# marekvinkler/NTrace

Measured on AMD Instinct MI355X. Metric: Mrays/sec (primary + 8xAO) on Crytek Sponza, higher is better.
Workload: dtype f32

## Files before the change

### include/ntrace_amd.h

```cpp
#ifndef NTRACE_AMD_H
#define NTRACE_AMD_H

#include <stddef.h>
#include <stdint.h>

#ifdef __cplusplus
extern "C" {
#endif

#define NTR_API __attribute__((visibility("default")))

typedef enum NtrStatus {
    NTR_OK = 0,
    NTR_ERR_INVALID = -1,
    NTR_ERR_NO_DEVICE = -2,
    NTR_ERR_HIP = -3,
    NTR_ERR_LAYOUT = -4,
    NTR_ERR_UNKNOWN_KERNEL = -5,
    NTR_ERR_OVERFLOW = -6,
    NTR_ERR_NOMEM = -7
} NtrStatus;

typedef enum NtrBVHLayout {
    NTR_BVHLayout_AOS_AOS = 0,
// ... 5 lines not shown
    NTR_BVHLayout_CPU,
    NTR_BVHLayout_Max
} NtrBVHLayout;

typedef struct NtrKernelConfig {
    int32_t bvhLayout;
    int32_t blockWidth;
    int32_t blockHeight;
    int32_t usePersistentThreads;
} NtrKernelConfig;

typedef struct NtrRay {
    float ox, oy, oz, tmin;
    float dx, dy, dz, tmax;
} NtrRay;

typedef struct NtrRayResult {
    int32_t id;
    float   t;
    int32_t padA;
    int32_t padB;
} NtrRayResult;


NTR_API const char* ntr_last_error(void);
NTR_API int         ntr_version(void);

NTR_API int ntr_device_count(int* count);
NTR_API int ntr_set_device(int device);
NTR_API int ntr_malloc(void** d_ptr, size_t bytes);
NTR_API int ntr_free(void* d_ptr);
NTR_API int ntr_memcpy_h2d(void* d_dst, const void* h_src, size_t bytes, void* stream);
NTR_API int ntr_memcpy_d2h(void* h_dst, const void* d_src, size_t bytes, void* stream);
NTR_API int ntr_memcpy_d2d(void* d_dst, const void* d_src, size_t bytes, void* stream);
NTR_API int ntr_memset(void* d_dst, int value, size_t bytes, void* stream);
NTR_API int ntr_stream_synchronize(void* stream);


NTR_API int ntr_query_config(const char* kernelName, NtrKernelConfig* config);

NTR_API int ntr_trace_bvh(const char* kernelName, int32_t numRays, int32_t anyHit,
                          const NtrRay* d_rays, NtrRayResult* d_results,
                          const void* d_nodes, int64_t nodesBytes,
                          const void* d_triWoop, int64_t triWoopBytes, const int32_t* d_triIndex,
                          int32_t layout, uint32_t bvhFlags, void* stream, float* seconds);

NTR_API int ntr_trace_status(void* stream, uint32_t* statusBits);

NTR_API int ntr_selftest_gather_rate(int64_t tableBytes, int32_t waves, int32_t lanesPerWave, int32_t steps, void* stream, float* seconds);

NTR_API int ntr_trace_graph_reserve(int32_t launches, int32_t numRays);
NTR_API int ntr_trace_graph_release_all(void);

NTR_API int ntr_stream_release(void* stream);

NTR_API int ntr_selftest_auto_hint_table(int32_t devices, int32_t keysPerDevice, int32_t rounds, int32_t* hintedLastRound);

typedef struct NtrTracePlan {
    int32_t variant;
    int32_t launchVariant;
    int32_t launchBlocks;
    int32_t numBlocks;
    int32_t orderBlocks;
    int32_t chunk, fetchThreshold, leafSwitchBelow, octant, flatFetch, uniformPrologue, splitSlice;
    int32_t numHeads, shardRays, numBlocksIncoherent;
    int32_t numBlocksDivergent;
    int32_t wholeWave;
    int32_t prefetchAfter;
    int32_t unified;
    int32_t minipool;
    int32_t poolKConst;
    int32_t poolKFromDevice;
    int32_t minipoolWide;
    int32_t hintable;
    int32_t useAutoHint;
    int32_t predictable;
    int32_t persistentOrder;
    int32_t probeOnRefresh;
    int32_t coherentRoute;
    int32_t persistentVariant, persistentBlocks, persistentFetchThreshold;
    int32_t perrayBlocks, perrayFetchThreshold;
} NtrTracePlan;
#define NTR_PLAN_FLAG_STATS 1
#define NTR_PLAN_FLAG_CAPTURING 2
#define NTR_PLAN_FLAG_CALLER_HINT 4
NTR_API int ntr_trace_plan(const char* kernelName, int32_t numRays, int32_t anyHit, uint64_t nodesAddr, int64_t nodesBytes,
                           uint64_t triWoopAddr, int64_t triWoopBytes, uint32_t bvhFlags, int32_t numCUs, int32_t flags,
                           NtrTracePlan* plan);
NTR_API int ntr_trace_plan_hint_step(int32_t valid, int32_t predicted, int32_t uses, int32_t out[3]);
NTR_API int ntr_trace_plan_certain(int32_t anyHit, int32_t out[2]);

NTR_API int ntr_tunables_reload(void);

typedef struct NtrSchedHint NtrSchedHint;
NTR_API int ntr_sched_hint_create(NtrSchedHint** out);
NTR_API int ntr_sched_hint_destroy(NtrSchedHint* hint);
NTR_API int ntr_sched_hint_reset(NtrSchedHint* hint);
NTR_API int ntr_trace_bvh_hinted(const char* kernelName, int32_t numRays, int32_t anyHit,
                                 const NtrRay* d_rays, NtrRayResult* d_results,
                                 const void* d_nodes, int64_t nodesBytes,
                                 const void* d_triWoop, int64_t triWoopBytes, const int32_t* d_triIndex,
                                 int32_t layout, uint32_t bvhFlags, void* stream, float* seconds,
                                 NtrSchedHint* hint);

NTR_API int ntr_sched_hint_predict(NtrSchedHint* hint, const uint32_t* d_blockCost, int32_t numBlocks, void* stream);
NTR_API int ntr_bvh_leaf_depths(const void* d_nodes, int64_t nodesBytes, const void* d_triWoop, int64_t triWoopBytes,
                                const int32_t* d_triIndex, int32_t numTris, int32_t* d_depthByTri, int32_t* levels, void* stream);
NTR_API int ntr_secondary_block_costs(const NtrRayResult* d_inResults, int32_t first, int32_t count, int32_t numSamples,
                                      const int32_t* d_depthByTri, int32_t numTris, uint32_t* d_blockCost, void* stream);

NTR_API int ntr_predict_block_costs(int32_t numRays, const NtrRay* d_rays, const void* d_nodes, int64_t nodesBytes,
                                    uint32_t* d_blockCost, void* stream);

NTR_API int ntr_predict_batch_coherence(int32_t numRays, const NtrRay* d_rays, const void* d_nodes, int64_t nodesBytes,
                                        uint32_t* d_out, void* stream);

NTR_API int ntr_predict_dispatch_order(int32_t numRays, const NtrRay* d_rays, const void* d_nodes, int64_t nodesBytes,
                                       uint32_t* d_order, uint32_t* d_word, void* stream);

typedef struct {
    int32_t numBlocks;
    int32_t device;
    int32_t uses;
    int32_t valid;
    int32_t predicted;
} NtrSchedHintState;
NTR_API int ntr_sched_hint_inspect(const NtrSchedHint* hint, NtrSchedHintState* state, uint32_t* h_order, uint32_t* h_cost, void* stream);

typedef struct NtrTraceStats {
    int64_t numRays;
    int64_t numInnerVisits;
    int64_t numTriTests;
    int64_t numLeafVisits;
    int64_t numHits;
} NtrTraceStats;

NTR_API int ntr_trace_bvh_stats(const char* kernelName, int32_t numRays, int32_t anyHit,
                                const NtrRay* d_rays, NtrRayResult* d_results,
                                const void* d_nodes, int64_t nodesBytes,
                                const void* d_triWoop, int64_t triWoopBytes, const int32_t* d_triIndex,
                                int32_t layout, uint32_t bvhFlags, void* stream, NtrTraceStats* stats);

#define NTR_BVH_FINITE 1u
#define NTR_BVH_FASTDIV 2u
#define NTR_BVH_NOTINY 4u
#define NTR_BVH_ORDERED 8u
#define NTR_BVH_WIDE_LEAVES 16u
#define NTR_BATCH_DIVERGENT 0x10000u
NTR_API int ntr_bvh_validate(const void* d_nodes, int64_t nodesBytes, uint32_t* flags, void* stream);

NTR_API int ntr_selftest_division(const float* d_x, int32_t nx, const float* d_d, int32_t nd,
                                  uint32_t* mismatches, void* stream);
NTR_API int ntr_selftest_division_hard(int32_t xExp, int32_t dExp, uint64_t* pairs, uint64_t* mismatches, void* stream);


NTR_API int ntr_pixel_table(int32_t w, int32_t h, int32_t* d_indexToPixel, int32_t* d_pixelToIndex, void* stream);

NTR_API int ntr_raygen_primary(NtrRay* d_rays, int32_t* d_idToSlot, int32_t* d_slotToID,
                               const int32_t* d_indexToPixel, const float origin[3],
                               const float nscreenToWorld[16], int32_t w, int32_t h, float maxDist,
                               uint32_t kernelSeed, void* stream);

NTR_API int ntr_raygen_ao(NtrRay* d_outRays, int32_t* d_outIDToSlot, int32_t* d_outSlotToID,
                          const NtrRay* d_inRays, const NtrRayResult* d_inResults,
                          const float* d_triNormals, int32_t firstInputSlot, int32_t numInputRays,
                          int32_t numSamples, float maxDist, uint32_t kernelSeed, void* stream);

NTR_API int ntr_raygen_ao_normals(NtrRay* d_outRays, int32_t* d_outIDToSlot, int32_t* d_outSlotToID, const NtrRay* d_inRays,
                                  const NtrRayResult* d_inResults, const float* d_rayNormals ,
                                  int32_t firstInputSlot, int32_t numInputRays, int32_t numSamples, float maxDist,
                                  uint32_t kernelSeed, void* stream);

NTR_API int ntr_raygen_shadow(NtrRay* d_outRays, int32_t* d_outIDToSlot, int32_t* d_outSlotToID, const NtrRay* d_inRays,
                              const NtrRayResult* d_inResults, int32_t firstInputSlot, int32_t numInputRays, int32_t numSamples,
                              const float lightPos[3], float lightRadius, uint32_t kernelSeed, void* stream);

NTR_API int ntr_count_hits(const NtrRayResult* d_results, int32_t numRays, int32_t* count, void* stream);


typedef struct NtrLbvhResult {
    int32_t numNodes, numLeaves, numLevels, pad;
    int64_t nodesBytes, triWoopBytes, triIndexBytes;
    float   seconds;
    float   mortonMs, sortMs, woopMs, emitMs, refitMs;
} NtrLbvhResult;

NTR_API int ntr_lbvh_capacity(int32_t numTris, int64_t* nodesBytes, int64_t* triWoopBytes, int64_t* triIndexBytes);

NTR_API int ntr_lbvh_build(int32_t numTris, const int32_t* d_triVtxIndex, int32_t numVerts, const float* d_vtxPos,
                           const float sceneMin[3], const float sceneMax[3], int32_t leafSize, float epsilon,
                           void* d_nodes, int64_t nodesCapacity, void* d_triWoop, int64_t triWoopCapacity,
                           int32_t* d_triIndex, int64_t triIndexCapacity, NtrLbvhResult* result, void* stream);

typedef struct NtrHlbvhResult {
    NtrLbvhResult lbvh;
    int32_t numClusters, topNodes, topLevels, pad;
    float   clusterMs, topMs, bottomMs, pad2;
} NtrHlbvhResult;

NTR_API int ntr_hlbvh_build(int32_t numTris, const int32_t* d_triVtxIndex, int32_t numVerts, const float* d_vtxPos,
                            const float sceneMin[3], const float sceneMax[3], int32_t leafSize, float epsilon, int32_t hlbvhBits,
                            void* d_nodes, int64_t nodesCapacity, void* d_triWoop, int64_t triWoopCapacity,
                            int32_t* d_triIndex, int64_t triIndexCapacity, NtrHlbvhResult* result, void* stream);

NTR_API int ntr_lbvh_release_workspace(void);

typedef struct NtrPersistentBvhParams {
    int32_t triLimit, triMaxLimit, maxDepth, pad;
    float   ci, ct, epsilon, pad2;
} NtrPersistentBvhParams;
typedef struct NtrPersistentBvhResult {
    int32_t numNodes, numLeaves, numLevels, maxDepth;
    int32_t medianFallbacks, costLeaves, depthLeaves, pad;
    int64_t nodesBytes, triWoopBytes, triIndexBytes;
    float   seconds;
    float   prepMs, levelsMs, emitMs;
} NtrPersistentBvhResult;
NTR_API int ntr_persistent_bvh_params_default(NtrPersistentBvhParams* params);
NTR_API int ntr_persistent_bvh_build(int32_t numTris, const int32_t* d_triVtxIndex, int32_t numVerts, const float* d_vtxPos,
                                     const float sceneMin[3], const float sceneMax[3], const NtrPersistentBvhParams* params,
                                     void* d_nodes, int64_t nodesCapacity, void* d_triWoop, int64_t triWoopCapacity,
                                     int32_t* d_triIndex, int64_t triIndexCapacity, NtrPersistentBvhResult* result, void* stream);
NTR_API int ntr_persistent_bvh_scratch_bytes(int64_t* bytes);

typedef struct NtrSahDeviceResult {
    int32_t numNodes, numLeaves, numLevels, maxDepth;
    int32_t numDropped, pad[3];
    int64_t nodesBytes, triWoopBytes, triIndexBytes;
    float   seconds;
    float   prepMs, sortMs, levelsMs, emitMs;
} NtrSahDeviceResult;
NTR_API int ntr_sah_device_build(int32_t numTris, const int32_t* d_triVtxIndex, int32_t numVerts, const float* d_vtxPos,
                                 int32_t minLeafSize, int32_t maxLeafSize, void* d_nodes, int64_t nodesCapacity, void* d_triWoop,
                                 int64_t triWoopCapacity, int32_t* d_triIndex, int64_t triIndexCapacity, NtrSahDeviceResult* result,
                                 void* stream);
NTR_API int ntr_sah_device_scratch_bytes(int64_t* bytes);

#define NTR_PLOC_TAIL 1024
#define NTR_PLOC_TILE 1024
typedef struct NtrPlocResult {
    int32_t numNodes, numLeaves, numRounds, height;
    int32_t tailClusters, pad[3];
    int64_t nodesBytes, triWoopBytes, triIndexBytes;
    float   seconds;
    float   mortonMs, sortMs, roundsMs, tailMs, emitMs;
} NtrPlocResult;
NTR_API int ntr_ploc_build(int32_t numTris, const int32_t* d_triVtxIndex, int32_t numVerts, const float* d_vtxPos,
                           const float sceneMin[3], const float sceneMax[3], int32_t radius, void* d_nodes, int64_t nodesCapacity,
                           void* d_triWoop, int64_t triWoopCapacity, int32_t* d_triIndex, int64_t triIndexCapacity, NtrPlocResult* result,
                           void* stream);
NTR_API int ntr_ploc_scratch_bytes(int64_t* bytes);

typedef struct NtrBlasRange { int64_t nodesOffset, nodesBytes, triWoopOffset, triWoopBytes; } NtrBlasRange;
typedef struct NtrInstance {
    float   objectToWorld[12];
    float   worldToObject[12];
    int32_t blas;
    int32_t reserved[3];
} NtrInstance;
typedef struct NtrTlasResult {
    int32_t rootLink, numNodes, numRounds, height;
    int32_t tailClusters, pad[3];
    int64_t nodesBytes, recordsBytes;
    float   sceneMin[3], sceneMax[3];
    float   seconds;
    float   boxesMs, sortMs, clustersMs, roundsMs, tailMs;
} NtrTlasResult;
NTR_API int ntr_instance_invert(const float objectToWorld[12], float worldToObject[12]);
NTR_API int ntr_tlas_capacity(int32_t numInstances, int64_t* nodesBytes, int64_t* recordsBytes);
NTR_API int ntr_tlas_build(int32_t numInstances, const NtrInstance* d_instances, int32_t numBlas, const NtrBlasRange* blasRanges,
                           const void* d_poolNodes, int64_t poolNodesBytes, int32_t radius, void* d_tlasNodes, int64_t tlasNodesCapacity,
                           void* d_records, int64_t recordsCapacity, NtrTlasResult* result, void* stream);
NTR_API int ntr_tlas_scratch_bytes(int64_t* bytes);
NTR_API int ntr_trace_instanced(int32_t numRays, int32_t anyHit, const NtrRay* d_rays, NtrRayResult* d_results, int32_t* d_instanceIDs,
                                const void* d_tlasNodes, int64_t tlasNodesBytes, int32_t rootLink, const void* d_records,
                                int32_t numInstances, const void* d_poolNodes, int64_t poolNodesBytes, const void* d_poolTriWoop,
                                int64_t poolTriWoopBytes, const int32_t* d_poolTriIndex, float* seconds ,
                                void* stream);

typedef struct NtrInstanceVisibility {
    const uint32_t* d_instanceMasks;
    const uint32_t* d_rayMasks;
    uint32_t rayMask, pad;
} NtrInstanceVisibility;
typedef struct NtrInstancedTraceStats {
    int64_t numRays;
    int64_t numTopInnerVisits;
    int64_t numInstanceEntries;
    int64_t numInstancesMasked;
    int64_t numInnerVisits;
    int64_t numTriTests;
    int64_t numLeafVisits;
    int64_t numHits;
} NtrInstancedTraceStats;
NTR_API int ntr_trace_instanced_masked(int32_t numRays, int32_t anyHit, const NtrRay* d_rays, NtrRayResult* d_results, int32_t* d_instanceIDs,
                                       const void* d_tlasNodes, int64_t tlasNodesBytes, int32_t rootLink, const void* d_records,
                                       int32_t numInstances, const void* d_poolNodes, int64_t poolNodesBytes, const void* d_poolTriWoop,
                                       int64_t poolTriWoopBytes, const int32_t* d_poolTriIndex,
                                       const NtrInstanceVisibility* vis , float* seconds ,
                                       void* stream);
NTR_API int ntr_trace_instanced_stats(int32_t numRays, int32_t anyHit, const NtrRay* d_rays, NtrRayResult* d_results, int32_t* d_instanceIDs,
                                      const void* d_tlasNodes, int64_t tlasNodesBytes, int32_t rootLink, const void* d_records,
                                      int32_t numInstances, const void* d_poolNodes, int64_t poolNodesBytes, const void* d_poolTriWoop,
                                      int64_t poolTriWoopBytes, const int32_t* d_poolTriIndex,
                                      const NtrInstanceVisibility* vis , NtrInstancedTraceStats* stats, void* stream);

// ... 246 lines not shown
```

### ntrace_amd/__init__.py

```python
from ._capi import (BvhView, RAY_DTYPE, RESULT_DTYPE, HostBvh, KernelConfig, NtrError, TraceStats, bvh_validate, lib,
                    lib_path, query_config, sah_build, trace_bvh, trace_bvh_stats, pixel_table,
                    raygen_primary, raygen_ao, raygen_shadow, count_hits, selftest_division, selftest_division_hard, bvh_leaf_depths, secondary_block_costs, lbvh_capacity,
                    lbvh_build, LbvhResult, hlbvh_build, HlbvhResult, reconstruct, ray_morton_sort, camera_decode, camera_reencode,
                    camera_nscreen_to_world, obj_load, SchedHint, trace_status, trace_plan, trace_plan_hint_step, trace_plan_certain, TracePlan, set_tunables, host_bvh_wrap, use_library, trace_graph_reserve, trace_graph_release_all, stream_release, selftest_auto_hint_table, selftest_gather_rate, frame_shard, frame_ao_batches, DistGroup,
                    lbvh_release_workspace, predict_block_costs, predict_batch_coherence, predict_dispatch_order, SchedHintState,
                    HostKdtree, kdtree_build, host_kdtree_wrap, trace_kdtree, KDTREE_SPATIAL_MEDIAN, KDTREE_SAH,
                    DeviceKdtree, KdtreeDeviceParams, kdtree_device_build, kdtree_device_params, KDTREE_DEVICE_DEFAULTS,
                    kdtree_device_scratch_bytes, PersistentBvhParams, PersistentBvhResult, persistent_bvh_params,
                    persistent_bvh_build, persistent_bvh_scratch_bytes, PERSISTENT_BVH_DEFAULTS, SahDeviceResult,
                    sah_device_build, sah_device_scratch_bytes, BvhRefitResult, bvh_refit,
                    bvh_refit_scratch_bytes, BvhOptimizeResult, BvhSahResult, bvh_optimize, bvh_optimize_scratch_bytes, bvh_sah_cost,
                    BvhReorderResult, bvh_reorder, bvh_reorder_scratch_bytes,
                    PlocResult, ploc_build, ploc_scratch_bytes, PLOC_TAIL, PLOC_TILE,
                    PlocBatchMesh, PlocBatchMeshResult, PlocBatchResult, ploc_batch_capacity, ploc_build_batch, ploc_batch_scratch_bytes,
                    RefitBatchEntry, BvhRefitBatchResult, bvh_refit_batch, bvh_refit_batch_scratch_bytes,
                    INSTANCE_DTYPE, BlasRange, BlasPool, TlasResult, instance_invert, make_instances, tlas_capacity, tlas_build,
                    tlas_scratch_bytes, trace_instanced, InstanceVisibility, InstancedTraceStats,
                    trace_instanced_masked, trace_instanced_stats, TlasRefitResult, tlas_refit, tlas_refit_scratch_bytes,
                    BlasTris, BLAS_TRIS_DTYPE, InstancedGeometry, instanced_hit_attributes, raygen_ao_normals,
                    BvhWideResult, bvh_widen_capacity, bvh_widen, bvh_widen_scratch_bytes, trace_wide, trace_wide_stats)

BVHLayout_Compact = 4
BVH_FINITE, BVH_FASTDIV, BVH_NOTINY, BVH_ORDERED, BVH_WIDE_LEAVES = 1, 2, 4, 8, 16
KERNELS = ("fermi_speculative_while_while", "tesla_persistent_while_while",
           "tesla_persistent_speculative_while_while", "kepler_dynamic_fetch")

__all__ = ["BvhView", "RAY_DTYPE", "RESULT_DTYPE", "HostBvh", "KernelConfig", "NtrError", "bvh_validate", "lib",
           "lib_path", "query_config", "sah_build", "trace_bvh", "trace_bvh_stats", "TraceStats", "pixel_table", "raygen_primary", "raygen_ao", "count_hits", "selftest_division", "selftest_division_hard", "bvh_leaf_depths", "secondary_block_costs", "lbvh_capacity", "lbvh_build", "LbvhResult", "hlbvh_build", "HlbvhResult", "reconstruct", "ray_morton_sort", "camera_decode", "camera_reencode", "camera_nscreen_to_world", "obj_load", "SchedHint", "trace_status", "set_tunables", "host_bvh_wrap", "BVHLayout_Compact", "KERNELS",
           "HostKdtree", "kdtree_build", "host_kdtree_wrap", "trace_kdtree", "KDTREE_SPATIAL_MEDIAN", "KDTREE_SAH",
           "DeviceKdtree", "KdtreeDeviceParams", "kdtree_device_build", "kdtree_device_params", "KDTREE_DEVICE_DEFAULTS",
           "kdtree_device_scratch_bytes", "PersistentBvhParams", "PersistentBvhResult", "persistent_bvh_params",
           "persistent_bvh_build", "persistent_bvh_scratch_bytes", "PERSISTENT_BVH_DEFAULTS", "SahDeviceResult",
           "sah_device_build", "sah_device_scratch_bytes", "BvhRefitResult", "bvh_refit",
           "bvh_refit_scratch_bytes", "BvhOptimizeResult", "BvhSahResult", "bvh_optimize", "bvh_optimize_scratch_bytes",
           "bvh_sah_cost", "BvhReorderResult", "bvh_reorder", "bvh_reorder_scratch_bytes",
           "PlocResult", "ploc_build", "ploc_scratch_bytes", "PLOC_TAIL", "PLOC_TILE",
           "PlocBatchMesh", "PlocBatchMeshResult", "PlocBatchResult", "ploc_batch_capacity", "ploc_build_batch", "ploc_batch_scratch_bytes",
           "RefitBatchEntry", "BvhRefitBatchResult", "bvh_refit_batch", "bvh_refit_batch_scratch_bytes",
           "INSTANCE_DTYPE", "BlasRange", "BlasPool", "TlasResult", "instance_invert", "make_instances", "tlas_capacity", "tlas_build",
           "tlas_scratch_bytes", "trace_instanced", "InstanceVisibility", "InstancedTraceStats",
           "trace_instanced_masked", "trace_instanced_stats", "TlasRefitResult", "tlas_refit", "tlas_refit_scratch_bytes",
           "BlasTris", "BLAS_TRIS_DTYPE", "InstancedGeometry", "instanced_hit_attributes", "raygen_ao_normals",
           "BvhWideResult", "bvh_widen_capacity", "bvh_widen", "bvh_widen_scratch_bytes", "trace_wide", "trace_wide_stats"]
```

### ntrace_amd/_capi.py

```python
import ctypes as C
import os

import numpy as np

_HERE = os.path.dirname(os.path.abspath(__file__))

RAY_DTYPE = np.dtype([("ox", "<f4"), ("oy", "<f4"), ("oz", "<f4"), ("tmin", "<f4"),
                      ("dx", "<f4"), ("dy", "<f4"), ("dz", "<f4"), ("tmax", "<f4")])
RESULT_DTYPE = np.dtype([("id", "<i4"), ("t", "<f4"), ("padA", "<i4"), ("padB", "<i4")])


class NtrError(RuntimeError):
    def __init__(self, code, msg):
        super().__init__("ntrace_amd error %d: %s" % (code, msg))
        self.code = code


class SchedHintState(C.Structure):
    _fields_ = [(n, C.c_int32) for n in ("numBlocks", "device", "uses", "valid", "predicted")]


class KernelConfig(C.Structure):
    _fields_ = [("bvhLayout", C.c_int32), ("blockWidth", C.c_int32), ("blockHeight", C.c_int32),
                ("usePersistentThreads", C.c_int32)]
# ... 154 lines not shown
    _fields_ = [("numEntries", C.c_int32), ("lanesPerLeaf", C.c_int32), ("numNodes", C.c_int64), ("numLeaves", C.c_int64),
                ("numRows", C.c_int64), ("firstBadEntry", C.c_int32), ("errBits", C.c_int32), ("seconds", C.c_float), ("pad", C.c_float)]

    def as_dict(self):
        return {k: getattr(self, k) for k, _ in self._fields_ if k != "pad"}


class BlasTris(C.Structure):
    _fields_ = [("firstTri", C.c_int32), ("numTris", C.c_int32)]


BLAS_TRIS_DTYPE = np.dtype([("firstTri", "<i4"), ("numTris", "<i4")])


class InstancedGeometry(C.Structure):
    _fields_ = [("numInstances", C.c_int32), ("numBlas", C.c_int32), ("numTrisTotal", C.c_int32), ("numVerts", C.c_int32),
                ("d_instances", C.c_void_p), ("d_blasTris", C.c_void_p), ("d_triVtxIndex", C.c_void_p), ("d_vtxPos", C.c_void_p)]

    def __init__(self, num_instances=0, num_blas=0, num_tris_total=0, num_verts=0, d_instances=0, d_blas_tris=0, d_tri=0, d_pos=0):
        super().__init__(int(num_instances), int(num_blas), int(num_tris_total), int(num_verts), int(d_instances) or None,
                         int(d_blas_tris) or None, int(d_tri) or None, int(d_pos) or None)


class TlasResult(C.Structure):
    _fields_ = [("rootLink", C.c_int32), ("numNodes", C.c_int32), ("numRounds", C.c_int32), ("height", C.c_int32),
                ("tailClusters", C.c_int32), ("pad", C.c_int32 * 3), ("nodesBytes", C.c_int64), ("recordsBytes", C.c_int64),
                ("sceneMin", C.c_float * 3), ("sceneMax", C.c_float * 3), ("seconds", C.c_float), ("boxesMs", C.c_float),
                ("sortMs", C.c_float), ("clustersMs", C.c_float), ("roundsMs", C.c_float), ("tailMs", C.c_float)]

    def as_dict(self):
        return {k: (list(getattr(self, k)) if k.startswith("scene") else getattr(self, k)) for k, _ in self._fields_ if k != "pad"}


class TlasRefitResult(C.Structure):
    _fields_ = [("numNodes", C.c_int32), ("numLeaves", C.c_int32), ("errBits", C.c_int32), ("pad", C.c_int32),
                ("sceneMin", C.c_float * 3), ("sceneMax", C.c_float * 3), ("seconds", C.c_float), ("pad2", C.c_float)]

    def as_dict(self):
        return {k: (list(getattr(self, k)) if k.startswith("scene") else getattr(self, k)) for k, _ in self._fields_ if not k.startswith("pad")}


class BvhWideResult(C.Structure):
    _fields_ = [("nodesBytes", C.c_int64), ("numNodes", C.c_int32), ("counts", C.c_int32 * 3), ("numLeafLinks", C.c_int32),
                ("height", C.c_int32), ("stackBound", C.c_int32), ("seconds", C.c_float)]

    def as_dict(self):
        return {k: (list(getattr(self, k)) if k == "counts" else getattr(self, k)) for k, _ in self._fields_}


class BvhRefitResult(C.Structure):
    _fields_ = [("numNodes", C.c_int32), ("numLeaves", C.c_int32), ("numRows", C.c_int32), ("pad", C.c_int32), ("seconds", C.c_float)]

    def as_dict(self):
        return {k: getattr(self, k) for k, _ in self._fields_ if k != "pad"}


class BvhOptimizeResult(C.Structure):
    _fields_ = [("passes", C.c_int32), ("numNodes", C.c_int32), ("numLeafLinks", C.c_int32), ("pad", C.c_int32),
                ("formed", C.c_int32 * 8), ("rewritten", C.c_int32 * 8), ("heightBefore", C.c_int32 * 8), ("heightAfter", C.c_int32 * 8),
                ("seconds", C.c_float)]

    def as_dict(self):
        n = self.passes
        return {k: (list(getattr(self, k))[:n] if k in ("formed", "rewritten", "heightBefore", "heightAfter") else getattr(self, k))
                for k, _ in self._fields_ if k != "pad"}


class BvhReorderResult(C.Structure):
    _fields_ = [("nodesBytes", C.c_int64), ("triWoopBytes", C.c_int64), ("triIndexBytes", C.c_int64),
                ("numNodes", C.c_int32), ("numLeaves", C.c_int32), ("numRows", C.c_int32), ("numDroppedSlots", C.c_int32),
                ("seconds", C.c_float)]

    def as_dict(self):
        return {k: getattr(self, k) for k, _ in self._fields_}


class BvhSahResult(C.Structure):
    _fields_ = [("sahCost", C.c_float), ("numNodes", C.c_int32), ("numLeaves", C.c_int32), ("numTris", C.c_int32), ("height", C.c_int32),
                ("seconds", C.c_float)]

    def as_dict(self):
        return {k: getattr(self, k) for k, _ in self._fields_}


class _DeviceKdtreeInfo(C.Structure):
    _fields_ = [("nodes", C.c_void_p), ("nodesBytes", C.c_int64), ("triWoop", C.c_void_p),
                ("triWoopBytes", C.c_int64), ("triIndex", C.c_void_p), ("triIndexBytes", C.c_int64),
                ("sceneMin", C.c_float * 3), ("sceneMax", C.c_float * 3), ("delta", C.c_float),
                ("numInnerNodes", C.c_int32), ("numLeafNodes", C.c_int32), ("numEmptyLeaves", C.c_int32), ("numTriRefs", C.c_int32),
                ("maxDepth", C.c_int32), ("numLevels", C.c_int32), ("percentDuplicates", C.c_float), ("seconds", C.c_float),
                ("prepMs", C.c_float), ("levelsMs", C.c_float), ("emitMs", C.c_float)]


def lib_path():
    return os.environ.get("NTR_LIB_OVERRIDE") or os.path.join(_HERE, "libntrace_amd.so")


_lib = None
_libs = {}

_vp, _i32, _i64, _u32 = C.c_void_p, C.c_int32, C.c_int64, C.c_uint32
SYMBOLS = [
    ("ntr_last_error", C.c_char_p, []),
    ("ntr_version", C.c_int, []),
    ("ntr_device_count", C.c_int, [C.POINTER(C.c_int)]),
    ("ntr_set_device", C.c_int, [C.c_int]),
    ("ntr_malloc", C.c_int, [C.POINTER(_vp), C.c_size_t]),
    ("ntr_free", C.c_int, [_vp]),
    ("ntr_memcpy_h2d", C.c_int, [_vp, _vp, C.c_size_t, _vp]),
    ("ntr_memcpy_d2h", C.c_int, [_vp, _vp, C.c_size_t, _vp]),
    ("ntr_memcpy_d2d", C.c_int, [_vp, _vp, C.c_size_t, _vp]),
    ("ntr_memset", C.c_int, [_vp, C.c_int, C.c_size_t, _vp]),
    ("ntr_stream_synchronize", C.c_int, [_vp]),
    ("ntr_query_config", C.c_int, [C.c_char_p, C.POINTER(KernelConfig)]),
    ("ntr_trace_bvh", C.c_int, [C.c_char_p, _i32, _i32, _vp, _vp, _vp, _i64, _vp, _i64, _vp, _i32, _u32, _vp,
                                C.POINTER(C.c_float)]),
    ("ntr_trace_bvh_hinted", C.c_int, [C.c_char_p, _i32, _i32, _vp, _vp, _vp, _i64, _vp, _i64, _vp, _i32, _u32, _vp,
                                       C.POINTER(C.c_float), _vp]),
    ("ntr_trace_status", C.c_int, [_vp, C.POINTER(_u32)]),
    ("ntr_trace_plan", C.c_int, [C.c_char_p, _i32, _i32, C.c_uint64, _i64, C.c_uint64, _i64, _u32, _i32, _i32, _vp]),
    ("ntr_trace_plan_hint_step", C.c_int, [_i32, _i32, _i32, C.POINTER(_i32 * 3)]),
    ("ntr_trace_plan_certain", C.c_int, [_i32, C.POINTER(_i32 * 2)]),
    ("ntr_selftest_gather_rate", C.c_int, [_i64, _i32, _i32, _i32, _vp, C.POINTER(C.c_float)]),
    ("ntr_frame_shard", C.c_int, [_i32, _i32, _i32, _i32, C.POINTER(_i32), C.POINTER(_i32)]),
    ("ntr_frame_ao_batches", C.c_int, [_i32, _i32, _i32, _i32, C.POINTER(_i32), C.POINTER(_i32), _i32, C.POINTER(_i32)]),
    ("ntr_dist_unique_id", C.c_int, [C.c_char_p]),
    ("ntr_dist_init", C.c_int, [C.c_char_p, _i32, _i32, C.POINTER(_vp)]),
    ("ntr_dist_init_all", C.c_int, [_i32, C.POINTER(_i32), C.POINTER(_vp)]),
    ("ntr_dist_info", C.c_int, [_vp, C.POINTER(_i32), C.POINTER(_i32)]),
    ("ntr_dist_destroy", C.c_int, [_vp]),
    ("ntr_dist_broadcast", C.c_int, [_vp, _vp, _i64, _i32, _vp]),
    ("ntr_dist_broadcast_bvh", C.c_int, [_vp, _vp, _i64, _vp, _i64, _vp, _i64, _i32, _vp]),
    ("ntr_dist_gather_records", C.c_int, [_vp, _vp, _i32, _i32, _vp, _i32, _vp]),
    ("ntr_dist_gather_records_cuts", C.c_int, [_vp, _vp, C.POINTER(_i32), _vp, _i32, _vp]),
    ("ntr_dist_gather_pixels", C.c_int, [_vp, _vp, _vp, _i32, _i32, _vp, _vp, _i32, _vp]),
    ("ntr_tunables_reload", C.c_int, []),
    ("ntr_predict_block_costs", C.c_int, [_i32, _vp, _vp, _i64, _vp, _vp]),
    ("ntr_predict_batch_coherence", C.c_int, [_i32, _vp, _vp, _i64, _vp, _vp]),
    ("ntr_predict_dispatch_order", C.c_int, [_i32, _vp, _vp, _i64, _vp, _vp, _vp]),
    ("ntr_trace_graph_reserve", C.c_int, [_i32, _i32]),
    ("ntr_trace_graph_release_all", C.c_int, []),
    ("ntr_stream_release", C.c_int, [_vp]),
    ("ntr_selftest_auto_hint_table", C.c_int, [_i32, _i32, _i32, C.POINTER(_i32)]),
    ("ntr_lbvh_release_workspace", C.c_int, []),
    ("ntr_sched_hint_create", C.c_int, [C.POINTER(_vp)]),
    ("ntr_sched_hint_destroy", C.c_int, [_vp]),
    ("ntr_sched_hint_reset", C.c_int, [_vp]),
    ("ntr_sched_hint_predict", C.c_int, [_vp, _vp, _i32, _vp]),
    ("ntr_sched_hint_inspect", C.c_int, [_vp, _vp, _vp, _vp, _vp]),
    ("ntr_secondary_block_costs", C.c_int, [_vp, _i32, _i32, _i32, _vp, _i32, _vp, _vp]),
    ("ntr_bvh_leaf_depths", C.c_int, [_vp, _i64, _vp, _i64, _vp, _i32, _vp, C.POINTER(_i32), _vp]),
    ("ntr_selftest_division", C.c_int, [_vp, _i32, _vp, _i32, C.POINTER(_u32), _vp]),
    ("ntr_selftest_division_hard", C.c_int, [_i32, _i32, C.POINTER(C.c_uint64), C.POINTER(C.c_uint64), _vp]),
    ("ntr_trace_bvh_stats", C.c_int, [C.c_char_p, _i32, _i32, _vp, _vp, _vp, _i64, _vp, _i64, _vp, _i32, _u32, _vp,
                                      C.POINTER(TraceStats)]),
    ("ntr_bvh_validate", C.c_int, [_vp, _i64, C.POINTER(_u32), _vp]),
    ("ntr_pixel_table", C.c_int, [_i32, _i32, _vp, _vp, _vp]),
    ("ntr_raygen_primary", C.c_int, [_vp, _vp, _vp, _vp, C.POINTER(C.c_float), C.POINTER(C.c_float), _i32, _i32,
                                     C.c_float, _u32, _vp]),
    ("ntr_raygen_ao", C.c_int, [_vp, _vp, _vp, _vp, _vp, _vp, _i32, _i32, _i32, C.c_float, _u32, _vp]),
    ("ntr_raygen_ao_normals", C.c_int, [_vp, _vp, _vp, _vp, _vp, _vp, _i32, _i32, _i32, C.c_float, _u32, _vp]),
    ("ntr_raygen_shadow", C.c_int, [_vp, _vp, _vp, _vp, _vp, _i32, _i32, _i32, C.POINTER(C.c_float * 3), C.c_float, _u32, _vp]),
    ("ntr_count_hits", C.c_int, [_vp, _i32, C.POINTER(_i32), _vp]),
    ("ntr_lbvh_capacity", C.c_int, [_i32, C.POINTER(_i64), C.POINTER(_i64), C.POINTER(_i64)]),
    ("ntr_lbvh_build", C.c_int, [_i32, _vp, _i32, _vp, C.POINTER(C.c_float), C.POINTER(C.c_float), _i32, C.c_float,
                                 _vp, _i64, _vp, _i64, _vp, _i64, C.POINTER(LbvhResult), _vp]),
    ("ntr_hlbvh_build", C.c_int, [_i32, _vp, _i32, _vp, C.POINTER(C.c_float), C.POINTER(C.c_float), _i32, C.c_float, _i32,
                                  _vp, _i64, _vp, _i64, _vp, _i64, C.POINTER(HlbvhResult), _vp]),
    ("ntr_reconstruct", C.c_int, [_i32, _i32, _i32, _i32, _vp, _vp, _vp, _vp, _vp, _vp, _vp, _vp]),
    ("ntr_ray_morton_sort", C.c_int, [_i32, _vp, _vp, _vp, _vp, _vp, _vp, C.POINTER(C.c_float)]),
    ("ntr_camera_decode", C.c_int, [C.c_char_p, C.POINTER(C.c_float)]),
    ("ntr_camera_reencode", C.c_int, [C.c_char_p, C.c_char_p, _i32]),
    ("ntr_camera_nscreen_to_world", C.c_int, [C.c_char_p, _i32, _i32, C.POINTER(C.c_float), C.POINTER(C.c_float),
                                              C.POINTER(C.c_float)]),
    ("ntr_obj_load", C.c_int, [C.c_char_p, C.POINTER(_vp), C.POINTER(_i32), C.POINTER(_i32), C.POINTER(_i32)]),
    ("ntr_obj_get", C.c_int, [_vp, _vp, _vp]),
    ("ntr_obj_free", None, [_vp]),
    ("ntr_sah_build", C.c_int, [_i32, _vp, _i32, _vp, _i32, _i32, C.POINTER(_vp)]),
    ("ntr_host_bvh_info", C.c_int, [_vp, C.POINTER(_HostBvhInfo)]),
    ("ntr_host_bvh_free", None, [_vp]),
    ("ntr_host_bvh_wrap", C.c_int, [_vp, _i64, _vp, _i64, _vp, _i64, C.POINTER(_vp)]),
    ("ntr_host_bvh_trace", C.c_int, [_vp, _i32, _i32, _vp, _vp, _vp, _i32, C.POINTER(TraceStats)]),
    ("ntr_kdtree_build", C.c_int, [_i32, _i32, _vp, _i32, _vp, _i32, C.POINTER(_vp)]),
    ("ntr_kdtree_device_params_default", C.c_int, [C.POINTER(KdtreeDeviceParams)]),
    ("ntr_kdtree_device_build", C.c_int, [_i32, _vp, _i32, _vp, C.POINTER(KdtreeDeviceParams), C.POINTER(_vp), _vp]),
    ("ntr_device_kdtree_info", C.c_int, [_vp, C.POINTER(_DeviceKdtreeInfo)]),
    ("ntr_device_kdtree_free", None, [_vp]),
    ("ntr_device_kdtree_download", C.c_int, [_vp, _vp, _vp, _vp]),
    ("ntr_kdtree_device_scratch_bytes", C.c_int, [C.POINTER(_i64)]),
    ("ntr_persistent_bvh_params_default", C.c_int, [C.POINTER(PersistentBvhParams)]),
    ("ntr_persistent_bvh_build", C.c_int, [_i32, _vp, _i32, _vp, C.POINTER(C.c_float), C.POINTER(C.c_float), C.POINTER(PersistentBvhParams),
                                           _vp, _i64, _vp, _i64, _vp, _i64, C.POINTER(PersistentBvhResult), _vp]),
    ("ntr_persistent_bvh_scratch_bytes", C.c_int, [C.POINTER(_i64)]),
    ("ntr_sah_device_build", C.c_int, [_i32, _vp, _i32, _vp, _i32, _i32, _vp, _i64, _vp, _i64, _vp, _i64, C.POINTER(SahDeviceResult), _vp]),
    ("ntr_sah_device_scratch_bytes", C.c_int, [C.POINTER(_i64)]),
    ("ntr_ploc_build", C.c_int, [_i32, _vp, _i32, _vp, C.POINTER(C.c_float), C.POINTER(C.c_float), _i32, _vp, _i64, _vp, _i64, _vp, _i64,
                                 C.POINTER(PlocResult), _vp]),
    ("ntr_ploc_scratch_bytes", C.c_int, [C.POINTER(_i64)]),
    ("ntr_instance_invert", C.c_int, [_vp, _vp]),
    ("ntr_ploc_batch_capacity", C.c_int, [_i32, _vp, _vp, C.POINTER(_i64), C.POINTER(_i64), C.POINTER(_i64)]),
    ("ntr_ploc_build_batch", C.c_int, [_i32, _vp, _i32, _vp, _i32, _vp, _i32, _vp, _i64, _vp, _i64, _vp, _i64, _vp, _vp,
                                       C.POINTER(PlocBatchResult), _vp]),
    ("ntr_ploc_batch_scratch_bytes", C.c_int, [C.POINTER(_i64)]),
    ("ntr_tlas_capacity", C.c_int, [_i32, C.POINTER(_i64), C.POINTER(_i64)]),
    ("ntr_tlas_build", C.c_int, [_i32, _vp, _i32, _vp, _vp, _i64, _i32, _vp, _i64, _vp, _i64, C.POINTER(TlasResult), _vp]),
    ("ntr_tlas_scratch_bytes", C.c_int, [C.POINTER(_i64)]),
    ("ntr_tlas_refit", C.c_int, [_i32, _vp, _i32, _vp, _vp, _i64, _vp, _i64, _i32, _vp, _i64, _vp, C.POINTER(TlasRefitResult), _vp]),
    ("ntr_tlas_refit_scratch_bytes", C.c_int, [C.POINTER(_i64)]),
    ("ntr_trace_instanced", C.c_int, [_i32, _i32, _vp, _vp, _vp, _vp, _i64, _i32, _vp, _i32, _vp, _i64, _vp, _i64, _vp, C.POINTER(C.c_float), _vp]),
    ("ntr_trace_instanced_masked", C.c_int, [_i32, _i32, _vp, _vp, _vp, _vp, _i64, _i32, _vp, _i32, _vp, _i64, _vp, _i64, _vp,
                                             C.POINTER(InstanceVisibility), C.POINTER(C.c_float), _vp]),
    ("ntr_trace_instanced_stats", C.c_int, [_i32, _i32, _vp, _vp, _vp, _vp, _i64, _i32, _vp, _i32, _vp, _i64, _vp, _i64, _vp,
                                            C.POINTER(InstanceVisibility), C.POINTER(InstancedTraceStats), _vp]),
    ("ntr_instanced_hit_attributes", C.c_int, [_i32, _vp, _vp, C.POINTER(InstancedGeometry), _vp, _vp, _vp]),
    ("ntr_bvh_widen_capacity", C.c_int, [_i64, C.POINTER(_i64)]),
    ("ntr_bvh_widen", C.c_int, [_vp, _i64, _vp, _i64, C.POINTER(BvhWideResult), _vp]),
    ("ntr_bvh_widen_scratch_bytes", C.c_int, [C.POINTER(_i64)]),
    ("ntr_trace_wide", C.c_int, [_i32, _i32, _vp, _vp, _vp, _i64, _vp, _i64, _vp, _u32, _vp, C.POINTER(C.c_float)]),
    ("ntr_trace_wide_stats", C.c_int, [_i32, _i32, _vp, _vp, _vp, _i64, _vp, _i64, _vp, _u32, _vp, C.POINTER(TraceStats)]),
    ("ntr_bvh_refit", C.c_int, [_vp, _i64, _vp, _i64, _vp, _i64, _i32, _vp, _i32, _vp, C.c_float, _vp, C.POINTER(BvhRefitResult), _vp]),
    ("ntr_bvh_refit_scratch_bytes", C.c_int, [C.POINTER(_i64)]),
    ("ntr_bvh_refit_batch", C.c_int, [_i32, _vp, _vp, _i64, _vp, _i64, _vp, _i32, _vp, _i32, _vp, _vp, C.POINTER(BvhRefitBatchResult), _vp]),
    ("ntr_bvh_refit_batch_scratch_bytes", C.c_int, [C.POINTER(_i64)]),
    ("ntr_bvh_optimize", C.c_int, [_vp, _i64, _i32, C.POINTER(BvhOptimizeResult), _vp]),
    ("ntr_bvh_optimize_scratch_bytes", C.c_int, [C.POINTER(_i64)]),
    ("ntr_bvh_sah_cost", C.c_int, [_vp, _i64, _vp, _i64, C.POINTER(BvhSahResult), _vp]),
    ("ntr_bvh_reorder", C.c_int, [_vp, _i64, _vp, _i64, _vp, _i64, _vp, _i64, _vp, _i64, _vp, _i64, C.POINTER(BvhReorderResult), _vp]),
    ("ntr_bvh_reorder_scratch_bytes", C.c_int, [C.POINTER(_i64)]),
    ("ntr_host_kdtree_info", C.c_int, [_vp, C.POINTER(_HostKdtreeInfo)]),
    ("ntr_host_kdtree_free", None, [_vp]),
    ("ntr_host_kdtree_wrap", C.c_int, [_vp, _i64, _vp, _i64, _vp, _i64, C.POINTER(C.c_float), C.POINTER(C.c_float), C.POINTER(_vp)]),
    ("ntr_trace_kdtree", C.c_int, [_i32, _i32, C.POINTER(C.c_float), C.POINTER(C.c_float), _vp, _vp, _vp, _i64, _vp, _i64, _vp, _i64,
                                   _vp, C.POINTER(C.c_float)]),
]


def _load(path):
    if path not in _libs:
        if not os.path.exists(path):
            raise ImportError("ntrace_amd: %s not found -- run `python -c 'import __graft_entry__ as g; g.build()'` "
                              "(the HIP extension is mandatory; there is no CPU fallback)" % path)
        try:
            import torch
        except ImportError:
            pass
        L = C.CDLL(path)
        for name, res, args in SYMBOLS:
            fn = getattr(L, name)
            fn.restype = res
            fn.argtypes = args
        _libs[path] = L
    return _libs[path]


def lib():
    global _lib
    if _lib is None:
        _lib = _load(lib_path())
    return _lib


def use_library(path=None):
    global _lib
    _lib = _load(path or lib_path())
    return _lib


def _check(rc):
    if rc != 0:
        raise NtrError(rc, (lib().ntr_last_error() or b"").decode("utf-8", "replace"))


def query_config(kernel):
    cfg = KernelConfig()
    _check(lib().ntr_query_config(kernel.encode(), C.byref(cfg)))
    return cfg


class SchedHint:

    def __init__(self):
        self._h = _vp()
        _check(lib().ntr_sched_hint_create(C.byref(self._h)))

    def reset(self):
        _check(lib().ntr_sched_hint_reset(self._h))

    def predict(self, d_block_cost, num_blocks, stream=0):
        _check(lib().ntr_sched_hint_predict(self._h, _vp(d_block_cost), int(num_blocks), _vp(stream)))

    def inspect(self, stream=0):
        st = SchedHintState()
        _check(lib().ntr_sched_hint_inspect(self._h, C.byref(st), None, None, _vp(stream)))
        out = {n: int(getattr(st, n)) for n, _ in st._fields_}
        if st.numBlocks > 0:
            order = np.zeros(st.numBlocks + 3, np.uint32)
            cost = np.zeros(st.numBlocks, np.uint32)
            _check(lib().ntr_sched_hint_inspect(self._h, C.byref(st), order.ctypes.data_as(_vp), cost.ctypes.data_as(_vp), _vp(stream)))
            out.update({n: int(getattr(st, n)) for n, _ in st._fields_})
            out["order"], out["words"], out["cost"] = order[:st.numBlocks], order[st.numBlocks:], cost
        return out

    def close(self):
        if self._h:
            lib().ntr_sched_hint_destroy(self._h)
            self._h = _vp()
# ... 46 lines not shown
    _check(lib().ntr_trace_plan_hint_step(int(bool(valid)), int(bool(predicted)), int(uses), C.byref(out)))
    return dict(zeroK=bool(out[0]), refresh=bool(out[1]), useOrder=bool(out[2]))


def trace_plan_certain(any_hit):
    out = (_i32 * 2)()
    _check(lib().ntr_trace_plan_certain(int(bool(any_hit)), C.byref(out)))
    return dict(certainSteps=bool(out[0]), certainDescent=bool(out[1]))


def trace_status(stream=0):
    bits = _u32(0)
    _check(lib().ntr_trace_status(_vp(stream), C.byref(bits)))
    return int(bits.value)


def selftest_gather_rate(table_bytes, waves, lanes_per_wave=64, steps=256, stream=0):
    sec = C.c_float(0.0)
    _check(lib().ntr_selftest_gather_rate(int(table_bytes), int(waves), int(lanes_per_wave), int(steps), _vp(stream), C.byref(sec)))
    return float(sec.value)


def frame_shard(num_primary, rank, world, align=64):
    lo, hi = _i32(0), _i32(0)
    _check(lib().ntr_frame_shard(int(num_primary), int(rank), int(world), int(align), C.byref(lo), C.byref(hi)))
    return int(lo.value), int(hi.value)


def frame_ao_batches(lo, hi, samples, max_batch_rays):
    n = _i32(0)
    _check(lib().ntr_frame_ao_batches(int(lo), int(hi), int(samples), int(max_batch_rays), None, None, 0, C.byref(n)))
    first, count = (_i32 * max(n.value, 1))(), (_i32 * max(n.value, 1))()
    _check(lib().ntr_frame_ao_batches(int(lo), int(hi), int(samples), int(max_batch_rays), first, count, n.value, C.byref(n)))
    return [(int(first[i]), int(count[i])) for i in range(n.value)]


class DistGroup:

    @staticmethod
    def unique_id():
        buf = C.create_string_buffer(128)
        _check(lib().ntr_dist_unique_id(buf))
        return buf.raw

    def __init__(self, uid, rank, world, _handle=None):
        if _handle is not None:
            self._h, self.rank, self.world = _handle, int(rank), int(world)
            return
        h = _vp()
        _check(lib().ntr_dist_init(C.c_char_p(uid), int(rank), int(world), C.byref(h)))
        self._h, self.rank, self.world = h, int(rank), int(world)

    @staticmethod
    def init_all(devices):
        n = len(devices)
        devs = (_i32 * n)(*[int(x) for x in devices])
        hs = (_vp * n)()
        _check(lib().ntr_dist_init_all(n, devs, hs))
        return [DistGroup(None, i, n, _handle=_vp(hs[i])) for i in range(n)]

    def broadcast(self, d_buf, nbytes, root=0, stream=0):
        _check(lib().ntr_dist_broadcast(self._h, _vp(d_buf), int(nbytes), int(root), _vp(stream)))

    def broadcast_bvh(self, d_nodes, nodes_bytes, d_woop, woop_bytes, d_tri_index, tri_index_bytes, root=0, stream=0):
        _check(lib().ntr_dist_broadcast_bvh(self._h, _vp(d_nodes), int(nodes_bytes), _vp(d_woop), int(woop_bytes), _vp(d_tri_index), int(tri_index_bytes),
                                            int(root), _vp(stream)))

    def gather_records(self, d_own, num_primary, d_full, root=0, stream=0, align=64):
        _check(lib().ntr_dist_gather_records(self._h, _vp(d_own), int(num_primary), int(align), _vp(d_full), int(root), _vp(stream)))

    def gather_records_cuts(self, d_own, cuts, d_full, root=0, stream=0):
        if len(cuts) != self.world + 1:
            raise ValueError("gather_records_cuts: %d cut points for %d ranks" % (len(cuts), self.world))
        c = (_i32 * (self.world + 1))(*[int(x) for x in cuts])
        _check(lib().ntr_dist_gather_records_cuts(self._h, _vp(d_own), c, _vp(d_full), int(root), _vp(stream)))

    def gather_pixels(self, d_own_pixels, d_slot_to_pixel, num_primary, d_full_pixels, d_scratch, root=0, stream=0, align=64):
        _check(lib().ntr_dist_gather_pixels(self._h, _vp(d_own_pixels), _vp(d_slot_to_pixel), int(num_primary), int(align), _vp(d_full_pixels), _vp(d_scratch),
                                            int(root), _vp(stream)))

    def close(self):
        if self._h:
            lib().ntr_dist_destroy(self._h)
            self._h = None


def predict_batch_coherence(num_rays, d_rays, d_nodes, nodes_bytes, d_out, stream=0):
    _check(lib().ntr_predict_batch_coherence(int(num_rays), _vp(d_rays), _vp(d_nodes), int(nodes_bytes), _vp(d_out), _vp(stream)))


def predict_dispatch_order(num_rays, d_rays, d_nodes, nodes_bytes, d_order, d_word, stream=0):
    _check(lib().ntr_predict_dispatch_order(int(num_rays), _vp(d_rays), _vp(d_nodes), int(nodes_bytes), _vp(d_order), _vp(d_word), _vp(stream)))


def predict_block_costs(num_rays, d_rays, d_nodes, nodes_bytes, d_block_cost, stream=0):
    _check(lib().ntr_predict_block_costs(int(num_rays), _vp(d_rays), _vp(d_nodes), int(nodes_bytes), _vp(d_block_cost), _vp(stream)))


def trace_graph_reserve(launches, num_rays):
    _check(lib().ntr_trace_graph_reserve(int(launches), int(num_rays)))


def trace_graph_release_all():
    _check(lib().ntr_trace_graph_release_all())


def stream_release(stream=0):
    _check(lib().ntr_stream_release(_vp(stream)))


def selftest_auto_hint_table(devices, keys_per_device, rounds=3):
    out = (_i32 * devices)()
    _check(lib().ntr_selftest_auto_hint_table(devices, keys_per_device, rounds, out))
    return [int(x) for x in out]


def lbvh_release_workspace():
    _check(lib().ntr_lbvh_release_workspace())


def set_tunables(**kv):
    for k, v in kv.items():
        if v is None:
            os.environ.pop(k, None)
        else:
            os.environ[k] = str(v)
    _check(lib().ntr_tunables_reload())


def bvh_leaf_depths(d_nodes, nodes_bytes, d_woop, woop_bytes, d_tri_index, num_tris, d_depth_by_tri, stream=0):
    m = _i32(0)
    _check(lib().ntr_bvh_leaf_depths(_vp(d_nodes), int(nodes_bytes), _vp(d_woop), int(woop_bytes), _vp(d_tri_index), int(num_tris),
                                     _vp(d_depth_by_tri), C.byref(m), _vp(stream)))
    return int(m.value)


def secondary_block_costs(d_in_results, first, count, num_samples, d_depth_by_tri, num_tris, d_block_cost, stream=0):
    _check(lib().ntr_secondary_block_costs(_vp(d_in_results), int(first), int(count), int(num_samples), _vp(d_depth_by_tri), int(num_tris),
                                           _vp(d_block_cost), _vp(stream)))


def selftest_division(d_x, nx, d_d, nd, stream=0):
    m = _u32(0)
    _check(lib().ntr_selftest_division(_vp(d_x), int(nx), _vp(d_d), int(nd), C.byref(m), _vp(stream)))
    return int(m.value)


def selftest_division_hard(x_exp, d_exp, stream=0):
    n, m = C.c_uint64(0), C.c_uint64(0)
    _check(lib().ntr_selftest_division_hard(int(x_exp), int(d_exp), C.byref(n), C.byref(m), _vp(stream)))
    return int(n.value), int(m.value)


def trace_bvh_stats(kernel, num_rays, any_hit, d_rays, d_results, d_nodes, nodes_bytes, d_woop, woop_bytes,
                    d_tri_index, layout=4, bvh_flags=0, stream=0):
    st = TraceStats()
    _check(lib().ntr_trace_bvh_stats(kernel.encode(), int(num_rays), int(bool(any_hit)), _vp(d_rays), _vp(d_results),
                                     _vp(d_nodes), int(nodes_bytes), _vp(d_woop), int(woop_bytes), _vp(d_tri_index),
                                     int(layout), int(bvh_flags), _vp(stream), C.byref(st)))
    return st


def bvh_validate(d_nodes, nodes_bytes, stream=0):
    flags = _u32(0)
    _check(lib().ntr_bvh_validate(_vp(d_nodes), int(nodes_bytes), C.byref(flags), _vp(stream)))
    return int(flags.value)


def pixel_table(w, h, d_index_to_pixel, d_pixel_to_index=0, stream=0):
    _check(lib().ntr_pixel_table(int(w), int(h), _vp(d_index_to_pixel), _vp(d_pixel_to_index), _vp(stream)))


def raygen_primary(d_rays, d_id_to_slot, d_slot_to_id, d_index_to_pixel, origin, nscreen_to_world, w, h, max_dist,
                   kernel_seed=0, stream=0):
    o = (C.c_float * 3)(*[float(x) for x in origin])
    m = (C.c_float * 16)(*[float(x) for x in np.asarray(nscreen_to_world, dtype=np.float32).reshape(-1)])
    _check(lib().ntr_raygen_primary(_vp(d_rays), _vp(d_id_to_slot), _vp(d_slot_to_id), _vp(d_index_to_pixel), o, m,
                                    int(w), int(h), float(max_dist), int(kernel_seed), _vp(stream)))


def raygen_ao(d_out_rays, d_out_id_to_slot, d_out_slot_to_id, d_in_rays, d_in_results, d_tri_normals, first_input_slot,
              num_input_rays, num_samples, max_dist, kernel_seed=0, stream=0):
    _check(lib().ntr_raygen_ao(_vp(d_out_rays), _vp(d_out_id_to_slot), _vp(d_out_slot_to_id), _vp(d_in_rays),
                               _vp(d_in_results), _vp(d_tri_normals), int(first_input_slot), int(num_input_rays),
                               int(num_samples), float(max_dist), int(kernel_seed), _vp(stream)))


def raygen_ao_normals(d_out_rays, d_out_id_to_slot, d_out_slot_to_id, d_in_rays, d_in_results, d_ray_normals, first_input_slot,
                      num_input_rays, num_samples, max_dist, kernel_seed=0, stream=0):
    _check(lib().ntr_raygen_ao_normals(_vp(d_out_rays), _vp(d_out_id_to_slot), _vp(d_out_slot_to_id), _vp(d_in_rays),
                                       _vp(d_in_results), _vp(d_ray_normals), int(first_input_slot), int(num_input_rays),
                                       int(num_samples), float(max_dist), int(kernel_seed), _vp(stream)))


def raygen_shadow(d_out_rays, d_out_id_to_slot, d_out_slot_to_id, d_in_rays, d_in_results, first_input_slot, num_input_rays, num_samples,
                  light_pos, light_radius, kernel_seed=0, stream=0):
    lp = (C.c_float * 3)(*[float(x) for x in light_pos])
    _check(lib().ntr_raygen_shadow(_vp(d_out_rays), _vp(d_out_id_to_slot), _vp(d_out_slot_to_id), _vp(d_in_rays), _vp(d_in_results),
                                   int(first_input_slot), int(num_input_rays), int(num_samples), C.byref(lp), float(light_radius),
                                   int(kernel_seed), _vp(stream)))


def count_hits(d_results, num_rays, stream=0):
    cnt = _i32(0)
    _check(lib().ntr_count_hits(_vp(d_results), int(num_rays), C.byref(cnt), _vp(stream)))
    return int(cnt.value)


def reconstruct(ray_type, rays_per_primary, first_primary, num_primary, d_primary_slot_to_id, d_primary_results,
                d_batch_id_to_slot, d_batch_results, d_tri_material_color, d_tri_shaded_color, d_pixels, stream=0):
    _check(lib().ntr_reconstruct(int(ray_type), int(rays_per_primary), int(first_primary), int(num_primary),
                                 _vp(d_primary_slot_to_id), _vp(d_primary_results), _vp(d_batch_id_to_slot),
                                 _vp(d_batch_results), _vp(d_tri_material_color), _vp(d_tri_shaded_color), _vp(d_pixels),
                                 _vp(stream)))


def ray_morton_sort(num_rays, d_in_rays, d_in_slot_to_id, d_out_rays, d_out_id_to_slot, d_out_slot_to_id, stream=0):
    sec = C.c_float(0.0)
    _check(lib().ntr_ray_morton_sort(int(num_rays), _vp(d_in_rays), _vp(d_in_slot_to_id), _vp(d_out_rays),
                                     _vp(d_out_id_to_slot), _vp(d_out_slot_to_id), _vp(stream), C.byref(sec)))
    return float(sec.value)


def lbvh_capacity(num_tris):
    a, b, c = _i64(0), _i64(0), _i64(0)
    _check(lib().ntr_lbvh_capacity(int(num_tris), C.byref(a), C.byref(b), C.byref(c)))
    return int(a.value), int(b.value), int(c.value)


def lbvh_build(num_tris, d_tri, num_verts, d_pos, scene_min, scene_max, leaf_size, epsilon, d_nodes, nodes_cap,
               d_woop, woop_cap, d_idx, idx_cap, stream=0):
    res = LbvhResult()
    mn = (C.c_float * 3)(*[float(x) for x in scene_min])
    mx = (C.c_float * 3)(*[float(x) for x in scene_max])
    _check(lib().ntr_lbvh_build(int(num_tris), _vp(d_tri), int(num_verts), _vp(d_pos), mn, mx, int(leaf_size),
                                float(epsilon), _vp(d_nodes), int(nodes_cap), _vp(d_woop), int(woop_cap), _vp(d_idx),
                                int(idx_cap), C.byref(res), _vp(stream)))
    return res


def hlbvh_build(num_tris, d_tri, num_verts, d_pos, scene_min, scene_max, leaf_size, epsilon, hlbvh_bits, d_nodes, nodes_cap,
                d_woop, woop_cap, d_idx, idx_cap, stream=0):
    res = HlbvhResult()
    mn = (C.c_float * 3)(*[float(x) for x in scene_min])
    mx = (C.c_float * 3)(*[float(x) for x in scene_max])
    _check(lib().ntr_hlbvh_build(int(num_tris), _vp(d_tri), int(num_verts), _vp(d_pos), mn, mx, int(leaf_size), float(epsilon),
                                 int(hlbvh_bits), _vp(d_nodes), int(nodes_cap), _vp(d_woop), int(woop_cap), _vp(d_idx), int(idx_cap),
                                 C.byref(res), _vp(stream)))
    return res


PERSISTENT_BVH_DEFAULTS = dict(triLimit=16, triMaxLimit=16, maxDepth=50, ci=1.0, ct=1.0, epsilon=float(np.finfo(np.float32).eps))


def persistent_bvh_params(**kw):
    p = PersistentBvhParams()
    _check(lib().ntr_persistent_bvh_params_default(C.byref(p)))
    for k, v in kw.items():
        if k not in PERSISTENT_BVH_DEFAULTS:
            raise TypeError("unknown persistent BVH parameter %r" % k)
        setattr(p, k, v)
    return p


def persistent_bvh_build(num_tris, d_tri, num_verts, d_pos, scene_min, scene_max, d_nodes, nodes_cap, d_woop, woop_cap, d_idx, idx_cap,
                         params=None, stream=0):
    if isinstance(params, dict):
        params = persistent_bvh_params(**params)
    res = PersistentBvhResult()
    mn = (C.c_float * 3)(*[float(x) for x in scene_min])
    mx = (C.c_float * 3)(*[float(x) for x in scene_max])
    _check(lib().ntr_persistent_bvh_build(int(num_tris), _vp(d_tri), int(num_verts), _vp(d_pos), mn, mx,
                                          C.byref(params) if params is not None else None, _vp(d_nodes), int(nodes_cap), _vp(d_woop),
                                          int(woop_cap), _vp(d_idx), int(idx_cap), C.byref(res), _vp(stream)))
    return res


def persistent_bvh_scratch_bytes():
    v = _i64(0)
    _check(lib().ntr_persistent_bvh_scratch_bytes(C.byref(v)))
    return int(v.value)


def sah_device_build(num_tris, d_tri, num_verts, d_pos, d_nodes, nodes_cap, d_woop, woop_cap, d_idx, idx_cap, min_leaf=1, max_leaf=1,
                     stream=0):
    res = SahDeviceResult()
    _check(lib().ntr_sah_device_build(int(num_tris), _vp(d_tri), int(num_verts), _vp(d_pos), int(min_leaf), int(max_leaf), _vp(d_nodes),
                                      int(nodes_cap), _vp(d_woop), int(woop_cap), _vp(d_idx), int(idx_cap), C.byref(res), _vp(stream)))
    return res


def sah_device_scratch_bytes():
    v = _i64(0)
    _check(lib().ntr_sah_device_scratch_bytes(C.byref(v)))
    return int(v.value)


PLOC_TAIL, PLOC_TILE = 1024, 1024


def ploc_build(num_tris, d_tri, num_verts, d_pos, scene_min, scene_max, d_nodes, nodes_cap, d_woop, woop_cap, d_idx, idx_cap, radius=8,
               stream=0):
    res = PlocResult()
    mn = (C.c_float * 3)(*[float(x) for x in scene_min])
    mx = (C.c_float * 3)(*[float(x) for x in scene_max])
    _check(lib().ntr_ploc_build(int(num_tris), _vp(d_tri), int(num_verts), _vp(d_pos), mn, mx, int(radius), _vp(d_nodes), int(nodes_cap),
# ... 552 lines not shown
```

### ntrace_amd/csrc/ntr_api.cpp

```cpp

#include <hip/hip_runtime.h>

#include <cstdarg>
#include <cstdio>
#include <cstring>
#include <mutex>

#include "ntrace_amd.h"
#include "ntr_internal.h"
#include "compact_bvh.h"
#include "device_scratch.h"
#include "sched_state.h"
#include "trace_kernels.h"
#include "trace_plan.h"

namespace {

thread_local char g_err[512] = "";

}

namespace ntr {

int set_error(int code, const char* fmt, ...)
{
    va_list ap;
    va_start(ap, fmt);
    vsnprintf(g_err, sizeof(g_err), fmt, ap);
    va_end(ap);
    return code;
}

int hip_fail(hipError_t e, const char* what)
{
    int code = (e == hipErrorNoDevice || e == hipErrorInvalidDevice || e == hipErrorInsufficientDriver)
                   ? NTR_ERR_NO_DEVICE : NTR_ERR_HIP;
    return set_error(code, "%s: %s", what, hipGetErrorString(e));
}

bool stream_is_capturing(hipStream_t s)
{
    hipStreamCaptureStatus st = hipStreamCaptureStatusNone;
    if (hipStreamIsCapturing(s, &st) != hipSuccess) { (void)hipGetLastError(); return false; }
    return st != hipStreamCaptureStatusNone;
}

struct KernelInfo {
    const char* name;
    int variant;
    NtrKernelConfig cfg;
};

static const KernelInfo kKernels[] = {
    {"fermi_speculative_while_while", NTR_VARIANT_PERRAY,
     {NTR_BVHLayout_Compact, 64, 1, 0}},
    {"tesla_persistent_while_while", NTR_VARIANT_PERSISTENT,
     {NTR_BVHLayout_Compact, 64, NTR_TRACE_WAVES_PER_BLOCK, 1}},
    {"tesla_persistent_speculative_while_while", NTR_VARIANT_PERSISTENT,
     {NTR_BVHLayout_Compact, 64, NTR_TRACE_WAVES_PER_BLOCK, 1}},
    {"kepler_dynamic_fetch", NTR_VARIANT_PERSISTENT,
     {NTR_BVHLayout_Compact, 64, NTR_TRACE_WAVES_PER_BLOCK, 1}},
};

static const KernelInfo* find_kernel(const char* name)
{
    if (!name) return nullptr;
    for (const KernelInfo& k : kKernels)
        if (strcmp(k.name, name) == 0) return &k;
    return nullptr;
}

static TraceBatchDesc describe_batch(const KernelInfo* k, int32_t numRays, int32_t anyHit, uint64_t nodesAddr, int64_t nodesBytes,
                                     uint64_t woopAddr, int64_t triWoopBytes, uint32_t bvhFlags, bool wantStats, bool capturing,
                                     bool callerHint, int numCUs)
{
    TraceBatchDesc bd;
    bd.variant = k->variant; bd.dynamicFetch = strcmp(k->name, "kepler_dynamic_fetch") == 0;
    bd.numRays = numRays; bd.anyHit = anyHit != 0; bd.bvhFlags = bvhFlags;
    bd.nodesBytes = nodesBytes; bd.triWoopBytes = triWoopBytes;
    bd.nodesAddr = nodesAddr; bd.woopAddr = woopAddr;
    bd.wantStats = wantStats; bd.capturing = capturing; bd.callerHint = callerHint;
    bd.numCUs = numCUs;
    return bd;
}

struct TraceLaunch {
    TraceParams p{};
    TraceParams pp{};
    bool persistentSide = false, perraySide = false;
    NtrSchedHint* hint = nullptr;
    bool refresh = false;
    bool probeCoherence = false;
    TopTable* predTable = nullptr;
    PredictScratch* predScratch = nullptr;
};

static int bind_trace(DeviceState* ds, const Tunables& tun, const TracePlan& pl, bool capturing, int64_t nodesBytes, hipStream_t s,
                      NtrSchedHint* hint, TraceLaunch* L)
{
    TraceParams& p = L->p;
    const int variant = pl.variant, orderBlocks = pl.orderBlocks;
    int rc = NTR_OK;
    if (pl.useAutoHint) {
        rc = auto_hint_get(ds, p.rays, p.nodes, p.numRays, p.anyHit, s, orderBlocks, &hint);
        if (rc != NTR_OK) return rc;
    }
    L->hint = hint;
    if (hint && pl.hintable) {
        if (hint->numBlocks != orderBlocks || hint->device != ds->device) {
            rc = sched_hint_bind(hint, orderBlocks, ds->device, s);
            if (rc != NTR_OK) return rc;
        }
        const HintStep hs = plan_hint_step(tun, hint->valid, hint->predicted, hint->uses);
        if (hs.zeroK) {
            const hipError_t zk = ntr_launch_zero_words(hint->order + orderBlocks, 3, s);
            if (zk != hipSuccess) return hip_fail(zk, "zero_words launch");
        }
        L->refresh = hs.refresh;
        hint->predicted = false;
        hint->uses++;
        if (hs.useOrder) p.order = hint->order;
        if (L->refresh) {
            const hipError_t ze = ntr_launch_zero_words(hint->cost, orderBlocks, s);
            if (ze != hipSuccess) return hip_fail(ze, "zero_words launch");
            p.cost = hint->cost;
        }
    }

    if (pl.predictable && !(hint && hint->valid) && !p.order) {
        rc = top_table_get(ds, p.nodes, nodesBytes, s, false, &L->predTable);
        if (rc != NTR_OK) return rc;
        rc = predict_scratch_get(ds, s, orderBlocks, &L->predScratch);
        if (rc != NTR_OK) return rc;
        if (L->predScratch) p.order = (hint && pl.hintable) ? hint->order : L->predScratch->order;
        else L->predTable = nullptr;
    }

    L->probeCoherence = !L->predScratch && hint && L->refresh && pl.probeOnRefresh;
    if (L->probeCoherence) {
        rc = top_table_get(ds, p.nodes, nodesBytes, s, false, &L->predTable);
        if (rc != NTR_OK) return rc;
    }
    const unsigned int* word = nullptr;
    if (L->predScratch) word = L->predScratch->classCount + NTR_SCHED_PRED_CLASSES + 2;
    else if (hint && pl.hintable && hint->numBlocks == orderBlocks && hint->order) word = hint->order + orderBlocks + 2;
    const bool routed = pl.coherentRoute == 1 && word != nullptr;
    L->persistentSide = variant == NTR_VARIANT_PERSISTENT || routed;
    L->perraySide = variant != NTR_VARIANT_PERSISTENT || routed;
    if ((pl.minipool && pl.poolKFromDevice) || L->persistentSide) p.poolK = word;

    TraceParams& pp = L->pp = p;
    if (L->persistentSide) {
        rc = counter_set_take(ds, capturing, &pp.counter);
        if (rc != NTR_OK) return rc;
        pp.numBlocks = pl.persistentBlocks; pp.numBlocksIncoherent = pl.numBlocksIncoherent; pp.numBlocksDivergent = pl.numBlocksDivergent;
        pp.fetchThreshold = pl.persistentFetchThreshold;
        pp.shardRays = pl.shardRays;
        if (pp.order) {
            pp.orderBlocks = orderBlocks;
            pp.shardRays = ((orderBlocks + pp.numHeads - 1) / pp.numHeads) * 256;
        }
        pp.routeSkip = routed ? NTR_ROUTE_SKIP_COHERENT : 0;
    }
    if (routed) {
        p.routeSkip = NTR_ROUTE_SKIP_INCOHERENT;
        if (variant == NTR_VARIANT_PERSISTENT) { p.fetchThreshold = pl.perrayFetchThreshold; p.poolKConst = 1; }
    }
    return NTR_OK;
}

static int launch_trace(DeviceState* ds, const Tunables& tun, const TracePlan& pl, const TraceLaunch& L, hipStream_t s, float* seconds,
                        NtrTraceStats* stats)
{
    const TraceParams& p = L.p;
    NtrSchedHint* hint = L.hint;
    const int orderBlocks = pl.orderBlocks;
    StreamEvents<2> ev(s);
    if (seconds) {
        NTR_HIP(ev.create());
        NTR_HIP(hipStreamSynchronize(s));
        NTR_HIP(ev.record(0));
    }
    if (L.predScratch) {
        const hipError_t pe = ntr_launch_predict(p.rays, p.numRays, orderBlocks, L.predTable->table, L.predTable->count, L.predScratch->classCount,
                                                 L.predScratch->classList, (hint && pl.hintable) ? hint->order : L.predScratch->order,
                                                 (hint && pl.hintable) ? hint->order + orderBlocks + 2 : nullptr, pl.minipoolWide, s);
        if (pe != hipSuccess) return hip_fail(pe, "predict launch");
    } else if (L.probeCoherence) {
        const hipError_t ce = ntr_launch_coherence(p.rays, p.numRays, orderBlocks, L.predTable->table, L.predTable->count, hint->order + orderBlocks,
                                                  pl.minipoolWide, s);
        if (ce != hipSuccess) return hip_fail(ce, "coherence launch");
    }
    hipError_t le = hipSuccess;
    if (L.persistentSide) {
        le = ntr_launch_zero_words(L.pp.counter, kPoolHeadsMax * 16, s);
        if (le != hipSuccess) return hip_fail(le, "zero_words launch");
        le = ntr_launch_trace(pl.persistentVariant, &L.pp, pl.persistentBlocks, s);
        if (le != hipSuccess) return hip_fail(le, "trace_bvh launch");
    }
    if (L.perraySide) {
        le = pl.variant == NTR_VARIANT_PERSISTENT ? ntr_launch_trace(NTR_VARIANT_PERRAY_UNIFIED_MINI, &p, pl.perrayBlocks, s)
                                                  : ntr_launch_trace(pl.launchVariant, &p, pl.launchBlocks, s);
        if (le != hipSuccess) return hip_fail(le, "trace_bvh launch");
    }
    if (seconds) NTR_HIP(ev.record(1));
    if (L.refresh) {
        le = ntr_launch_sched_order(hint->cost, orderBlocks, tun.schedClasses, hint->order, 1, s);
        if (le != hipSuccess) return hip_fail(le, "sched_order launch");
        hint->valid = true;
    }
    if (seconds) {
        float ms = 0.0f;
        NTR_HIP(ev.elapsed(0, 1, &ms));
        *seconds = ms * 1e-3f;
        unsigned int st = 0;
        const int rc = status_fetch(ds, s, &st);
        if (rc != NTR_OK) return rc;
        if (st & NTR_STATUS_STACK_OVERFLOW) return set_error(NTR_ERR_OVERFLOW, "trace_bvh: traversal stack overflow");
    }
    if (stats) {
        unsigned long long h[4];
        NTR_HIP(hipMemcpyAsync(h, ds->stats, sizeof(h), hipMemcpyDeviceToHost, s));
        NTR_HIP(hipStreamSynchronize(s));
        stats->numRays = p.numRays;
        stats->numInnerVisits = (int64_t)h[0]; stats->numTriTests = (int64_t)h[1]; stats->numLeafVisits = (int64_t)h[2]; stats->numHits = (int64_t)h[3];
    }
    return NTR_OK;
}

static int32_t certain_steps_of(const Tunables& tun, bool anyHit) { return (tun.certainSteps >= 2 || (tun.certainSteps == 1 && anyHit)) ? 1 : 0; }

static int trace_impl(const char* kernelName, int32_t numRays, int32_t anyHit, const NtrRay* d_rays,
                      NtrRayResult* d_results, const void* d_nodes, int64_t nodesBytes, const void* d_triWoop,
                      int64_t triWoopBytes, const int32_t* d_triIndex, int32_t layout, uint32_t bvhFlags,
                      void* stream, float* seconds, NtrTraceStats* stats, NtrSchedHint* hint = nullptr)
{
    if (seconds) *seconds = 0.0f;
    if (stats) memset(stats, 0, sizeof(*stats));
    const KernelInfo* k = find_kernel(kernelName);
    if (!k) return set_error(NTR_ERR_UNKNOWN_KERNEL, "unknown kernel '%s'", kernelName ? kernelName : "(null)");
    if (numRays < 0) return set_error(NTR_ERR_INVALID, "ntr_trace_bvh: numRays < 0");
    if (numRays == 0) return NTR_OK;
    if (!d_nodes || !d_triWoop || !d_triIndex)
        return set_error(NTR_ERR_INVALID, "CudaBVHTracer: No BVH!");
    if (layout != k->cfg.bvhLayout)
        return set_error(NTR_ERR_LAYOUT, "CudaBVHTracer: Incorrect BVH layout!");
    if (!d_rays || !d_results) return set_error(NTR_ERR_INVALID, "ntr_trace_bvh: null ray/result buffer");
    int rc = check_nodes_bytes("ntr_trace_bvh", "node buffer size", nodesBytes);
    if (rc != NTR_OK) return rc;
    if (triWoopBytes < 16 || (triWoopBytes % 16) != 0 || triWoopBytes > 0xFFFFFFFFll)
        return set_error(NTR_ERR_INVALID, "ntr_trace_bvh: triWoop buffer size must be a multiple of 16 in [16, 4 GiB)");

    DeviceState* ds = nullptr;
    rc = current_device_state_ready(&ds);
    if (rc != NTR_OK) return rc;
    hipStream_t s = (hipStream_t)stream;

    const Tunables tun = tunables();
    const TraceBatchDesc bd = describe_batch(k, numRays, anyHit, (uint64_t)d_nodes, nodesBytes, (uint64_t)d_triWoop, triWoopBytes, bvhFlags,
                                             stats != nullptr, stream_is_capturing(s), hint != nullptr, ds->numCUs);
    const TracePlan pl = plan_trace(tun, bd);

    TraceLaunch L;
    TraceParams& p = L.p;
    p.numRays = numRays; p.anyHit = anyHit ? 1 : 0; p.rays = d_rays; p.results = d_results; p.bvhFlags = bvhFlags;
    p.nodes = d_nodes; p.woop = d_triWoop; p.triIndex = d_triIndex; p.nodesBytes = (uint32_t)nodesBytes; p.woopBytes = (uint32_t)triWoopBytes;
    p.status = ds->status; p.stats = ds->stats;
    p.numHeads = pl.numHeads; p.chunk = pl.chunk; p.fetchThreshold = pl.fetchThreshold; p.wholeWave = pl.wholeWave; p.prefetchAfter = pl.prefetchAfter;
    p.flatFetch = pl.flatFetch; p.uniformPrologue = pl.uniformPrologue; p.splitSlice = pl.splitSlice; p.leafSwitchBelow = pl.leafSwitchBelow;
    p.octant = pl.octant; p.poolKConst = pl.poolKConst;
    p.certainSteps = certain_steps_of(tun, anyHit != 0);
    p.certainDescent = tun.certainDescent != 0 ? 1 : 0;
    if (stats) NTR_HIP(hipMemsetAsync(ds->stats, 0, 4 * sizeof(unsigned long long), s));

    rc = bind_trace(ds, tun, pl, bd.capturing, nodesBytes, s, hint, &L);
    if (rc != NTR_OK) return rc;
    return launch_trace(ds, tun, pl, L, s, seconds, stats);
}

}

static int env_int(const char* name, int def)
{
    const char* v = getenv(name);
    return (v && *v) ? atoi(v) : def;
}

namespace ntr {
static Tunables g_tun;
static bool g_tunLoaded = false;
static std::mutex g_tunMu;

static void tunables_load_locked()
{
    Tunables t;
    t.chunk = env_int("NTR_TRACE_CHUNK", 64);
    t.fetchThreshold = env_int("NTR_TRACE_FETCH_THRESHOLD", -1);
    t.leafSwitchBelow = env_int("NTR_TRACE_LEAF_SWITCH", -1);
    t.blocksPerCU = env_int("NTR_TRACE_BLOCKS_PER_CU", 7);
    t.blocksPerCUIncoherent = env_int("NTR_TRACE_BLOCKS_PER_CU_INCOHERENT", 3);
    t.blocksPerCUDivergent = env_int("NTR_TRACE_BLOCKS_PER_CU_DIVERGENT", 4);
    t.octant = env_int("NTR_TRACE_OCTANT", 1);
    t.flatFetch = env_int("NTR_TRACE_FLAT_FETCH", 1);
    t.uniformPrologue = env_int("NTR_TRACE_UNIFORM_PROLOGUE", 1);
    t.certainSteps = env_int("NTR_TRACE_CERTAIN_STEPS", 1);
    t.certainDescent = env_int("NTR_TRACE_CERTAIN_DESCENT", 1);
    t.splitSlice = env_int("NTR_TRACE_SPLIT_SLICE", 8);
    t.wholeWave = env_int("NTR_TRACE_WHOLE_WAVE", 1);
    t.prefetchAfter = env_int("NTR_TRACE_PREFETCH_AFTER", 8);
    t.minipool = env_int("NTR_TRACE_MINIPOOL", -1);
    t.minipoolWide = env_int("NTR_TRACE_MINIPOOL_WIDE", -1);
    t.minipoolThreshold = env_int("NTR_TRACE_MINIPOOL_THRESHOLD", 48);
    t.unified = env_int("NTR_TRACE_UNIFIED", 1);
    t.poolHeads = env_int("NTR_TRACE_POOL_HEADS", 128);
    t.autoHint = env_int("NTR_TRACE_AUTO_HINT", 1);
    t.autoHintMinRays = env_int("NTR_TRACE_AUTO_HINT_MIN_RAYS", 1 << 17);
    t.route = env_int("NTR_TRACE_ROUTE", 1);
    t.persistentHints = env_int("NTR_TRACE_PERSISTENT_HINTS", 1);
    t.predict = env_int("NTR_TRACE_PREDICT", 1);
    t.predictPersistent = env_int("NTR_TRACE_PREDICT_PERSISTENT", 1);
// ... 176 lines not shown

static int query_table(const char* fn, const void* d_nodes, int64_t nodesBytes, hipStream_t s, DeviceState** ds, TopTable** t)
{
    int rc = check_nodes_bytes(fn, "node buffer size", nodesBytes);
    if (rc == NTR_OK) rc = current_device_state(ds, "hipGetDevice(&dev)");
    if (rc == NTR_OK) rc = top_table_get(*ds, d_nodes, nodesBytes, s, false, t);
    return rc;
}

int ntr_predict_block_costs(int32_t numRays, const NtrRay* d_rays, const void* d_nodes, int64_t nodesBytes, uint32_t* d_blockCost, void* stream)
{
    if (numRays < 0) return set_error(NTR_ERR_INVALID, "ntr_predict_block_costs: numRays < 0");
    if (numRays == 0) return NTR_OK;
    if (!d_rays || !d_nodes || !d_blockCost) return set_error(NTR_ERR_INVALID, "ntr_predict_block_costs: null argument");
    DeviceState* ds = nullptr;
    TopTable* t = nullptr;
    const int rc = query_table("ntr_predict_block_costs", d_nodes, nodesBytes, (hipStream_t)stream, &ds, &t);
    if (rc != NTR_OK) return rc;
    const hipError_t e = ntr_launch_predict_costs(d_rays, numRays, (numRays + 255) / 256, t->table, t->count, d_blockCost, (hipStream_t)stream);
    if (e != hipSuccess) return hip_fail(e, "predict_costs launch");
    return NTR_OK;
}

int ntr_predict_batch_coherence(int32_t numRays, const NtrRay* d_rays, const void* d_nodes, int64_t nodesBytes, uint32_t* d_out, void* stream)
{
    if (numRays < 0) return set_error(NTR_ERR_INVALID, "ntr_predict_batch_coherence: numRays < 0");
    if (!d_out) return set_error(NTR_ERR_INVALID, "ntr_predict_batch_coherence: null argument");
    if (numRays > 0 && (!d_rays || !d_nodes)) return set_error(NTR_ERR_INVALID, "ntr_predict_batch_coherence: null argument");
    if (numRays == 0) {
        const unsigned int none[3] = {0u, 0u, 1u};
        NTR_HIP(hipMemcpyAsync(d_out, none, sizeof(none), hipMemcpyHostToDevice, (hipStream_t)stream));
        NTR_HIP(hipStreamSynchronize((hipStream_t)stream));
        return NTR_OK;
    }
    DeviceState* ds = nullptr;
    TopTable* t = nullptr;
    const int rc = query_table("ntr_predict_batch_coherence", d_nodes, nodesBytes, (hipStream_t)stream, &ds, &t);
    if (rc != NTR_OK) return rc;
    const hipError_t e = ntr_launch_coherence(d_rays, numRays, (numRays + 255) / 256, t->table, t->count, d_out, minipool_wide(tunables(), nodesBytes, numRays),
                                              (hipStream_t)stream);
    if (e != hipSuccess) return hip_fail(e, "coherence launch");
    return NTR_OK;
}

int ntr_predict_dispatch_order(int32_t numRays, const NtrRay* d_rays, const void* d_nodes, int64_t nodesBytes, uint32_t* d_order, uint32_t* d_word,
                               void* stream)
{
    if (numRays < 0) return set_error(NTR_ERR_INVALID, "ntr_predict_dispatch_order: numRays < 0");
    if (numRays == 0) return NTR_OK;
    if (!d_rays || !d_nodes || !d_order || !d_word) return set_error(NTR_ERR_INVALID, "ntr_predict_dispatch_order: null argument");
    hipStream_t s = (hipStream_t)stream;
    DeviceState* ds = nullptr;
    TopTable* t = nullptr;
    int rc = query_table("ntr_predict_dispatch_order", d_nodes, nodesBytes, s, &ds, &t);
    if (rc != NTR_OK) return rc;
    std::lock_guard<std::mutex> lk(ds->queryMu);
    const int numBlocks = (numRays + 255) / 256;
    PredictScratch* p = &ds->query;
    if (p->capBlocks < numBlocks && p->classList) NTR_HIP(hipStreamSynchronize(s));
    rc = scratch_alloc(p, numBlocks);
    if (rc != NTR_OK) return rc;
    const hipError_t e = ntr_launch_predict(d_rays, numRays, numBlocks, t->table, t->count, p->classCount, p->classList, d_order, d_word,
                                            minipool_wide(tunables(), nodesBytes, numRays), s);
    if (e != hipSuccess) return hip_fail(e, "predict launch");
    NTR_HIP(hipStreamSynchronize(s));
    return NTR_OK;
}

int ntr_secondary_block_costs(const NtrRayResult* d_inResults, int32_t first, int32_t count, int32_t numSamples, const int32_t* d_depthByTri,
                              int32_t numTris, uint32_t* d_blockCost, void* stream)
{
    if (first < 0 || count < 0 || numSamples < 1 || numTris < 0 || (count > 0 && (!d_inResults || !d_depthByTri || !d_blockCost)))
        return set_error(NTR_ERR_INVALID, "ntr_secondary_block_costs: bad argument");
    if (count == 0) return NTR_OK;
    hipStream_t s = (hipStream_t)stream;
    const int64_t blocks = ((int64_t)count * numSamples + 255) / 256;
    if (blocks > 0x7FFFFFFF) return set_error(NTR_ERR_INVALID, "ntr_secondary_block_costs: batch too large");
    hipError_t e = ntr_launch_zero_words(d_blockCost, (int)blocks, s);
    if (e == hipSuccess) e = ntr_launch_secondary_block_costs(d_inResults, first, count, numSamples, d_depthByTri, numTris, d_blockCost, s);
    if (e != hipSuccess) return hip_fail(e, "secondary_block_costs launch");
    return NTR_OK;
}

int ntr_bvh_leaf_depths(const void* d_nodes, int64_t nodesBytes, const void* d_triWoop, int64_t triWoopBytes, const int32_t* d_triIndex,
                        int32_t numTris, int32_t* d_depthByTri, int32_t* maxDepth, void* stream)
{
    if (maxDepth) *maxDepth = 0;
    if (!d_nodes || nodesBytes < 64 || (nodesBytes % 64) != 0 || nodesBytes > kMaxNodesBytes || !d_triWoop || triWoopBytes < 16 || !d_triIndex ||
        numTris < 1 || !d_depthByTri)
        return set_error(NTR_ERR_INVALID, "ntr_bvh_leaf_depths: bad argument");
    hipStream_t s = (hipStream_t)stream;
    const unsigned int capacity = (unsigned int)(nodesBytes / 64);
    unsigned int* d_q = nullptr;
    NTR_HIP(hipMalloc((void**)&d_q, (2 * (size_t)capacity + 2) * sizeof(unsigned int)));
    unsigned int* q[2] = {d_q, d_q + capacity};
    unsigned int* cnt = d_q + 2 * (size_t)capacity;
    hipError_t e = hipMemsetAsync(d_depthByTri, 0, (size_t)numTris * sizeof(int32_t), s);
    const unsigned int init[3] = {0u, 1u, 0u};
    if (e == hipSuccess) e = hipMemcpyAsync(q[0], &init[0], sizeof(unsigned int), hipMemcpyHostToDevice, s);
    if (e == hipSuccess) e = hipMemcpyAsync(cnt, &init[1], 2 * sizeof(unsigned int), hipMemcpyHostToDevice, s);
    int depth = 0;
    unsigned long long bound = 1;
    unsigned int frontier = 1;
    while (e == hipSuccess && frontier > 0 && depth < 4096) {
        const int in = depth & 1, out = in ^ 1;
        e = ntr_launch_zero_words(cnt + out, 1, s);
        const unsigned int threads = (unsigned int)(bound < capacity ? bound : capacity);
        if (e == hipSuccess)
            e = ntr_launch_leaf_depth_level(d_nodes, (unsigned int)nodesBytes, d_triWoop, (unsigned int)(triWoopBytes / 16), d_triIndex, numTris, q[in], cnt + in,
                                            q[out], cnt + out, capacity, threads, depth, d_depthByTri, s);
        depth++;
        bound = bound < capacity ? bound * 2 : bound;
        if ((depth & 3) == 0 && e == hipSuccess) {
            e = hipMemcpyAsync(&frontier, cnt + (depth & 1), sizeof(frontier), hipMemcpyDeviceToHost, s);
            if (e == hipSuccess) e = hipStreamSynchronize(s);
            if (frontier > capacity) frontier = capacity;
        }
    }
    if (e == hipSuccess) e = hipStreamSynchronize(s);
    (void)hipFree(d_q);
    if (e != hipSuccess) return hip_fail(e, "ntr_bvh_leaf_depths");
    if (depth >= 4096) return set_error(NTR_ERR_INVALID, "ntr_bvh_leaf_depths: the tree is deeper than 4096 levels (a cycle in the child references?)");
    if (maxDepth) *maxDepth = depth;
    return NTR_OK;
}

int ntr_trace_bvh_stats(const char* kernelName, int32_t numRays, int32_t anyHit, const NtrRay* d_rays,
                        NtrRayResult* d_results, const void* d_nodes, int64_t nodesBytes, const void* d_triWoop,
                        int64_t triWoopBytes, const int32_t* d_triIndex, int32_t layout, uint32_t bvhFlags,
                        void* stream, NtrTraceStats* stats)
{
    if (!stats) return set_error(NTR_ERR_INVALID, "ntr_trace_bvh_stats: null stats");
    return trace_impl(kernelName, numRays, anyHit, d_rays, d_results, d_nodes, nodesBytes, d_triWoop, triWoopBytes,
                      d_triIndex, layout, bvhFlags, stream, nullptr, stats);
}

int ntr_selftest_division(const float* d_x, int32_t nx, const float* d_d, int32_t nd, uint32_t* mismatches, void* stream)
{
    if (!mismatches || !d_x || !d_d || nx <= 0 || nd <= 0) return set_error(NTR_ERR_INVALID, "ntr_selftest_division: bad argument");
    hipStream_t s = (hipStream_t)stream;
    unsigned int* d_m = nullptr;
    NTR_HIP(hipMalloc((void**)&d_m, sizeof(unsigned int)));
    NTR_HIP(hipMemsetAsync(d_m, 0, sizeof(unsigned int), s));
    hipError_t le = ntr_launch_selftest_division(d_x, d_d, nx, nd, d_m, s);
    if (le != hipSuccess) return hip_fail(le, "selftest launch");
    unsigned int m = 0;
    NTR_HIP(hipMemcpyAsync(&m, d_m, sizeof(m), hipMemcpyDeviceToHost, s));
    NTR_HIP(hipStreamSynchronize(s));
    NTR_HIP(hipFree(d_m));
    *mismatches = m;
    return NTR_OK;
}

int ntr_selftest_division_hard(int32_t xExp, int32_t dExp, uint64_t* pairs, uint64_t* mismatches, void* stream)
{
    if (!pairs || !mismatches || xExp < -84 || xExp > 51 || dExp < -40 || dExp > 16)
        return set_error(NTR_ERR_INVALID, "ntr_selftest_division_hard: bad argument (x exponents in [-84, 51], d exponents in [-40, 16])");
    hipStream_t s = (hipStream_t)stream;
    unsigned long long* d_c = nullptr;
    NTR_HIP(hipMalloc((void**)&d_c, 2 * sizeof(unsigned long long)));
    hipError_t e = hipMemsetAsync(d_c, 0, 2 * sizeof(unsigned long long), s);
    if (e == hipSuccess) e = ntr_launch_selftest_division_hard(xExp, dExp, d_c, s);
    unsigned long long h[2] = {0, 0};
    if (e == hipSuccess) e = hipMemcpyAsync(h, d_c, sizeof(h), hipMemcpyDeviceToHost, s);
    if (e == hipSuccess) e = hipStreamSynchronize(s);
    (void)hipFree(d_c);
    if (e != hipSuccess) return hip_fail(e, "ntr_selftest_division_hard");
    *pairs = h[0];
    *mismatches = h[1];
    return NTR_OK;
}

}
```

### ntrace_amd/csrc/selftest_kernels.hip

```cpp
#include <hip/hip_runtime.h>
#include <stdint.h>

#include "trace_kernels.h"
#include "trace_arith.h"

namespace ntr {

__global__ __launch_bounds__(256) void selftest_division_kernel(const float* __restrict__ x, const float* __restrict__ d,
                                                                int nx, int nd, unsigned int* __restrict__ mismatches)
{
    const int i = blockIdx.x * blockDim.x + threadIdx.x;
    if (i >= nx) return;
    const float xv = x[i];
    unsigned int bad = 0;
    for (int j = 0; j < nd; j++) {
        const float dv = d[j];
        const float q0 = xv / dv;
        const float q1 = fast_div(xv, dv, exact_rcp(dv));
        bad += (__float_as_uint(q0) != __float_as_uint(q1)) && !(q0 == 0.0f && q1 == 0.0f);
    }
    if (bad) atomicAdd(mismatches, bad);
}

__global__ __launch_bounds__(256) void selftest_division_hard_kernel(int xe0, int de0, unsigned long long* __restrict__ counts)
{
    const unsigned int D = (1u << 23) + blockIdx.x * 256u + threadIdx.x;
    const int k = __builtin_ctz(D);
    unsigned long long tested = 0, bad = 0;
    if (k <= 3) {
        const unsigned int Dp = D >> k;
        unsigned int inv = Dp;
        for (int it = 0; it < 5; it++) inv *= 2u - Dp * inv;
        for (int b = 24; b <= 25; b++) {
            const unsigned long long mod = 1ull << (b - k);
            for (int Np = -8; Np <= 8; Np++) {
                const long long N = (long long)Np * (1ll << k);
                if (Np == 0 || N > 8 || N < -8) continue;
                const unsigned long long base = ((unsigned long long)(unsigned int)(-Np) * inv) & (mod - 1ull);
                for (unsigned int j = 0; j < (1u << k); j++) {
                    unsigned long long Mo = base + j * mod;
                    while (Mo < (1ull << 24)) Mo += 1ull << b;
                    if (Mo >= (1ull << 25) || !(Mo & 1ull)) continue;
                    const long long num = (long long)((unsigned long long)D * Mo) + N;
                    if (num & ((1ll << b) - 1ll)) continue;
                    const long long X = num >> b;
                    if (b == 24 ? (X < (long long)D || X >= (1ll << 24)) : (X < (1ll << 23) || X >= (long long)D)) continue;
                    for (int e = 0; e < 16; e++) {
                        const float xv = ldexpf((float)X, xe0 + (e & 3) - 23), dv = ldexpf((float)D, de0 + (e >> 2) - 23);
                        for (int sgn = 0; sgn < 2; sgn++) {
                            const float dd = sgn ? -dv : dv;
                            const float q0 = xv / dd;
                            const float q1 = fast_div(xv, dd, exact_rcp(dd));
                            tested++;
                            bad += __float_as_uint(q0) != __float_as_uint(q1);
                        }
                    }
                }
            }
        }
    }
    if (tested) atomicAdd(&counts[0], tested);
    if (bad) atomicAdd(&counts[1], bad);
}

}

extern "C" hipError_t ntr_launch_selftest_division(const float* d_x, const float* d_d, int nx, int nd,
                                                   unsigned int* d_mismatches, hipStream_t stream)
{
    hipLaunchKernelGGL(ntr::selftest_division_kernel, dim3((nx + 255) / 256), dim3(256), 0, stream, d_x, d_d, nx, nd, d_mismatches);
    return hipGetLastError();
}

extern "C" hipError_t ntr_launch_selftest_division_hard(int xe0, int de0, unsigned long long* d_counts, hipStream_t stream)
{
    hipLaunchKernelGGL(ntr::selftest_division_hard_kernel, dim3((1u << 23) / 256u), dim3(256), 0, stream, xe0, de0, d_counts);
    return hipGetLastError();
}
```

### ntrace_amd/csrc/trace_fetch.h

```cpp
#pragma once
#include <hip/hip_runtime.h>
#include <stdint.h>

#include "trace_kernels.h"
#include "compact_bvh.h"

namespace ntr {

typedef __amdgpu_buffer_rsrc_t Rsrc;
typedef unsigned int u32x4 __attribute__((ext_vector_type(4)));
constexpr unsigned int kFetchBytes = kNodeBytes;

__device__ __forceinline__ Rsrc make_rsrc(const void* p, unsigned int bytes)
{
    return __builtin_amdgcn_make_buffer_rsrc(const_cast<void*>(p), 0, (int)bytes, 0x00020000);
}
__device__ __forceinline__ float4 as_f4(u32x4 v) { return make_float4(__uint_as_float(v.x), __uint_as_float(v.y), __uint_as_float(v.z), __uint_as_float(v.w)); }
__device__ __forceinline__ u32x4 as_u4(const float4& f) { return u32x4{__float_as_uint(f.x), __float_as_uint(f.y), __float_as_uint(f.z), __float_as_uint(f.w)}; }
__device__ __forceinline__ float4 ld4(Rsrc r, int byteOfs) { return as_f4(__builtin_amdgcn_raw_buffer_load_b128(r, byteOfs, 0, 0)); }
__device__ __forceinline__ unsigned int ld1(Rsrc r, int byteOfs)
{
    return __builtin_amdgcn_raw_buffer_load_b32(r, byteOfs, 0, 0);
}

__device__ __forceinline__ u32x4 rsrc_words(const void* p, unsigned int bytes)
{
    const unsigned long long a = (unsigned long long)p;
    u32x4 w;
    w.x = __builtin_amdgcn_readfirstlane((unsigned int)a);
    w.y = __builtin_amdgcn_readfirstlane((unsigned int)(a >> 32) & 0xFFFFu);
    w.z = __builtin_amdgcn_readfirstlane(bytes);
    w.w = 0x00020000u;
    return w;
}

#define NTR_FETCH64_TWO_BUFFERS_TEXT                                        \
    "s_mov_b64 %[sav], exec\n\t"                                            \
    "s_and_b64 exec, %[sav], %[ma]\n\t"                                     \
    "buffer_load_dwordx4 %[a], %[ofs], %[ra], 0 offen\n\t"                  \
    "buffer_load_dwordx4 %[b], %[ofs], %[ra], 0 offen offset:16\n\t"        \
    "buffer_load_dwordx4 %[c], %[ofs], %[ra], 0 offen offset:32\n\t"        \
    "buffer_load_dwordx4 %[d], %[ofs], %[ra], 0 offen offset:48\n\t"        \
    "s_and_b64 exec, %[sav], %[mb]\n\t"                                     \
    "buffer_load_dwordx4 %[a], %[ofs], %[rb], 0 offen\n\t"                  \
    "buffer_load_dwordx4 %[b], %[ofs], %[rb], 0 offen offset:16\n\t"        \
    "buffer_load_dwordx4 %[c], %[ofs], %[rb], 0 offen offset:32\n\t"        \
    "buffer_load_dwordx4 %[d], %[ofs], %[rb], 0 offen offset:48\n\t"        \
    "s_mov_b64 exec, %[sav]\n\t"                                            \
    "s_waitcnt vmcnt(0)"
#define NTR_FETCH64_TWO_BUFFERS_INPUTS [ofs] "v"(ofs), [ra] "s"(rsrcA), [rb] "s"(rsrcB), [ma] "s"(maskA), [mb] "s"(maskB)

__device__ __forceinline__ void fetch64_two_buffers(u32x4 rsrcA, u32x4 rsrcB, int ofs, unsigned long long maskA,
                                                    unsigned long long maskB, float4& a, float4& b, float4& c, float4& d)
{
    u32x4 va, vb, vc, vd;
    unsigned long long sav;
    asm volatile(NTR_FETCH64_TWO_BUFFERS_TEXT
                 : [a] "=&v"(va), [b] "=&v"(vb), [c] "=&v"(vc), [d] "=&v"(vd), [sav] "=&s"(sav)
                 : NTR_FETCH64_TWO_BUFFERS_INPUTS
                 : "memory", "scc");
    a = as_f4(va); b = as_f4(vb); c = as_f4(vc); d = as_f4(vd);
}

__device__ __forceinline__ void fetch64_two_buffers_into(u32x4 rsrcA, u32x4 rsrcB, int ofs, unsigned long long maskA,
                                                         unsigned long long maskB, float4& a, float4& b, float4& c, float4& d)
{
    u32x4 va = as_u4(a), vb = as_u4(b), vc = as_u4(c), vd = as_u4(d);
    unsigned long long sav;
    asm volatile(NTR_FETCH64_TWO_BUFFERS_TEXT
                 : [a] "+v"(va), [b] "+v"(vb), [c] "+v"(vc), [d] "+v"(vd), [sav] "=&s"(sav)
                 : NTR_FETCH64_TWO_BUFFERS_INPUTS
                 : "memory", "scc");
    a = as_f4(va); b = as_f4(vb); c = as_f4(vc); d = as_f4(vd);
}
#undef NTR_FETCH64_TWO_BUFFERS_TEXT
#undef NTR_FETCH64_TWO_BUFFERS_INPUTS

struct UnifiedBufs {
    const char* nodes; const char* woop;
    unsigned int nodesBytes, woopBytes;
    u32x4 rNodes, rWoop;
    bool uniformPrologue;
    bool certainSteps;
    bool certainDescent;
    const char* base;
    unsigned int dN, dW;
    unsigned int limNode;
    int limTri;
    unsigned int oddBase, oddSpan;
};
template <bool TRIM = false>
__device__ __forceinline__ UnifiedBufs unified_bufs(const TraceParams& p)
{
    UnifiedBufs u;
    u.nodes = (const char*)p.nodes; u.woop = (const char*)p.woop;
    u.nodesBytes = p.nodesBytes; u.woopBytes = p.woopBytes;
    u.rNodes = rsrc_words(p.nodes, p.nodesBytes); u.rWoop = rsrc_words(p.woop, p.woopBytes);
    u.uniformPrologue = p.uniformPrologue != 0;
    u.certainSteps = p.certainSteps != 0 && (p.bvhFlags & NTR_BVH_ORDERED) != 0;
    u.certainDescent = p.certainDescent != 0;
    const unsigned long long an = (unsigned long long)p.nodes, aw = (unsigned long long)p.woop;
    const unsigned long long lo = an < aw ? an : aw;
    u.base = (const char*)lo;
    u.dN = (unsigned int)(an - lo); u.dW = (unsigned int)(aw - lo);
    u.limNode = p.nodesBytes - kFetchBytes;
    u.limTri = leaf_link((int)((p.woopBytes - kFetchBytes) >> kRowShift));
    u.oddBase = u.limNode + 1u; u.oddSpan = (unsigned)u.limTri - u.oddBase;
    if (TRIM) asm volatile("" : "+s"(u.oddBase), "+s"(u.oddSpan));
    return u;
}

template <bool FLAT, bool TRIM = false>
__device__ __forceinline__ void unified_fetch(const UnifiedBufs& ub, int node, unsigned long long live, float4& a, float4& b, float4& c, float4& d)
{
    const bool inner = (unsigned)node < (unsigned)kSentinel;
    const bool atTri = node < 0;
    if (FLAT) {
        asm volatile("" : "=v"(a.x), "=v"(a.y), "=v"(a.z), "=v"(a.w), "=v"(b.x), "=v"(b.y), "=v"(b.z), "=v"(b.w));
        asm volatile("" : "=v"(c.x), "=v"(c.y), "=v"(c.z), "=v"(c.w), "=v"(d.x), "=v"(d.y), "=v"(d.z), "=v"(d.w));
        const bool okNode = (unsigned)node <= ub.limNode, okTri = TRIM ? (unsigned)node >= (unsigned)ub.limTri : atTri && node >= ub.limTri;
        const bool flatOk = okNode || okTri;
        const unsigned int cofs = okNode ? ub.dN + (unsigned)node : ub.dW + ((unsigned)leaf_row(node) << kRowShift);
        if (flatOk) {
            typedef const __attribute__((address_space(1))) u32x4* global_u4_ptr;
            const global_u4_ptr q = (global_u4_ptr)((const __attribute__((address_space(1))) char*)ub.base + cofs);
            const u32x4 qa = q[0], qb = q[1], qc = q[2], qd = q[3];
            a = as_f4(qa); b = as_f4(qb); c = as_f4(qc); d = as_f4(qd);
        }
        if (TRIM) {
            const unsigned long long odd = live & __builtin_amdgcn_ballot_w64((unsigned)node - ub.oddBase < ub.oddSpan);
            if (__builtin_expect(odd != 0ull, 0))
                fetch64_two_buffers_into(ub.rNodes, ub.rWoop, inner ? node : leaf_row(node) * kRowBytes, odd & __builtin_amdgcn_ballot_w64(inner),
                                         odd & __builtin_amdgcn_ballot_w64(atTri), a, b, c, d);
        } else {
            const unsigned long long odd = __ballot((inner || atTri) && !flatOk);
            if (odd != 0ull)
                fetch64_two_buffers_into(ub.rNodes, ub.rWoop, inner ? node : leaf_row(node) * kRowBytes, __ballot(inner && !flatOk), __ballot(atTri && !flatOk), a, b, c, d);
        }
    } else {
        const int ofs = inner ? node : leaf_row(node) * kRowBytes;
        fetch64_two_buffers(ub.rNodes, ub.rWoop, ofs, __ballot(inner), __ballot(atTri), a, b, c, d);
    }
}

}
```

### ntrace_amd/csrc/trace_kernels.h

```cpp
#pragma once
#include <hip/hip_runtime.h>
#include <stdint.h>

#include "ntrace_amd.h"

#ifndef NTR_TRACE_WAVES_PER_BLOCK
#define NTR_TRACE_WAVES_PER_BLOCK 4
#endif
#ifndef NTR_TRACE_MIN_WAVES_PER_SIMD
#define NTR_TRACE_MIN_WAVES_PER_SIMD 1
#endif
#ifndef NTR_TRACE_PERSISTENT_MIN_WAVES_PER_SIMD
#define NTR_TRACE_PERSISTENT_MIN_WAVES_PER_SIMD 1
#endif

#define NTR_VARIANT_PERRAY 0
#define NTR_VARIANT_PERSISTENT 1
#define NTR_VARIANT_PERRAY_STATS 2
#define NTR_VARIANT_PERSISTENT_UNIFIED 5
#define NTR_VARIANT_PERRAY_UNIFIED_W1 6
#define NTR_MINIPOOL_MAX_K 16
#define NTR_VARIANT_PERRAY_UNIFIED_MINI 7

#define NTR_ROUTE_SKIP_COHERENT 1
#define NTR_ROUTE_SKIP_INCOHERENT 2
#define NTR_BATCH_WORD_K(w) ((w) & 0xFFFFu)
#define NTR_BATCH_WORD_INCOHERENT(w) (NTR_BATCH_WORD_K(w) > 1u || ((w) & NTR_BATCH_DIVERGENT) != 0u)

#define NTR_STATUS_STACK_OVERFLOW 1u


namespace ntr {

struct TraceParams {
    int32_t numRays;
    int32_t anyHit;
    const NtrRay* rays;
    NtrRayResult* results;
    const void* nodes;
    const void* woop;
    uint32_t nodesBytes;
    uint32_t woopBytes;
    const int32_t* triIndex;
    int32_t* counter;
    unsigned int* status;
    int32_t chunk;
    int32_t shardRays;
    int32_t numHeads;
    int32_t numBlocks;
    int32_t numBlocksIncoherent;
    int32_t numBlocksDivergent;
    int32_t orderBlocks;
    int32_t fetchThreshold;
    int32_t wholeWave;
    int32_t prefetchAfter;
    uint32_t bvhFlags;
    int32_t leafSwitchBelow;
    int32_t octant;
    int32_t flatFetch;
    int32_t uniformPrologue;
    int32_t certainSteps;
    int32_t certainDescent;
    int32_t splitSlice;
    const unsigned int* order;
    unsigned int* cost;
    unsigned long long* stats;
    const unsigned int* poolK;
    int32_t poolKConst;
    int32_t routeSkip;
};

}

extern "C" hipError_t ntr_launch_trace(int variant, const ntr::TraceParams* p, int numBlocks, hipStream_t stream);
#define NTR_TOP_DEPTH_MAX 10
#define NTR_SCHED_PRED_CLASSES 64
#define NTR_SCHED_PRED_WORDS (NTR_SCHED_PRED_CLASSES + 3)
extern "C" hipError_t ntr_launch_top_table(const void* d_nodes, unsigned int nodesBytes, int depth, void* d_table,
                                           unsigned int* d_tableCount, hipStream_t stream);
extern "C" hipError_t ntr_launch_predict(const void* d_rays, int numRays, int numBlocks, const void* d_table,
                                         const unsigned int* d_tableCount, unsigned int* d_classCount, unsigned int* d_classList,
                                         unsigned int* d_order, unsigned int* d_poolKCopy, int poolKWide, hipStream_t stream);
extern "C" hipError_t ntr_launch_predict_costs(const void* d_rays, int numRays, int numBlocks, const void* d_table,
                                               const unsigned int* d_tableCount, unsigned int* d_blockCost, hipStream_t stream);
extern "C" hipError_t ntr_launch_coherence(const void* d_rays, int numRays, int numBlocks, const void* d_table, const unsigned int* d_tableCount,
                                           unsigned int* d_out, int poolKWide, hipStream_t stream);
extern "C" hipError_t ntr_launch_leaf_depth_level(const void* d_nodes, unsigned int nodesBytes, const void* d_woop, unsigned int woopVec4, const int* d_triIndex,
                                                  int numTris, const unsigned int* d_qin, const unsigned int* d_nIn, unsigned int* d_qout, unsigned int* d_nOut,
                                                  unsigned int capacity, unsigned int gridThreads, int depth, int* d_depthByTri, hipStream_t stream);
extern "C" hipError_t ntr_launch_secondary_block_costs(const void* d_inResults, int first, int count, int numSamples, const int* d_depthByTri, int numTris,
                                                       unsigned int* d_blockCost, hipStream_t stream);
extern "C" hipError_t ntr_launch_zero_words(void* d_ptr, int words, hipStream_t stream);
extern "C" hipError_t ntr_launch_status_exchange(unsigned int* d_status, unsigned int* d_out, hipStream_t stream);
extern "C" hipError_t ntr_launch_sched_order(const unsigned int* d_cost, int numBlocks, int classes, unsigned int* d_order,
                                             int keepIfAllZero, hipStream_t stream);
extern "C" hipError_t ntr_launch_identity_order(unsigned int* d_order, int numBlocks, hipStream_t stream);
extern "C" hipError_t ntr_launch_selftest_division(const float* d_x, const float* d_d, int nx, int nd,
                                                   unsigned int* d_mismatches, hipStream_t stream);
extern "C" hipError_t ntr_launch_selftest_division_hard(int xe0, int de0, unsigned long long* d_counts, hipStream_t stream);
```

### ntrace_amd/csrc/trace_kernels.hip

```cpp

#include <hip/hip_runtime.h>
#include <stdint.h>

#include "trace_kernels.h"
#include "trace_lane.h"
#include "trace_fetch.h"
#include "trace_prologue.h"
#include "trace_split.h"

namespace ntr {

template <bool FAST, bool STATS, bool DYNAMIC_FETCH, bool SLICED = false>
__device__ __forceinline__ void traverse(Rsrc nodes, Rsrc woop, RayRegs& r, int& node,
                                         LaneStack& st, int (&spill)[SPILL_DEPTH], bool anyHit,
                                         int& hitAddr, float& hitU, float& hitV, LaneStats& ls, unsigned int* status,
                                         bool poolEmpty, int fetchThreshold, int leafSwitchBelow, int* slice = nullptr)
{
    unsigned long long live = __ballot(node != kSentinel);
    while (live != 0ull) {
        if (SLICED && --*slice < 0) break;
        for (;;) {
            const bool inner = (unsigned)node < (unsigned)kSentinel;
            const unsigned long long innerMask = __ballot(inner);
            if (innerMask == 0ull) break;
            if (__popcll(innerMask) < leafSwitchBelow && __ballot(node < 0) != 0ull) break;
            inner_step<FAST>(nodes, inner, r, node, st, spill, status);
            if (STATS && inner) ls.inner++;
        }
        if (node < 0) {
            if (leaf_step<STATS>(woop, r, node, anyHit, hitAddr, hitU, hitV, ls)) node = kSentinel;
            else node = stack_pop(st, spill);
        }
        live = __ballot(node != kSentinel);
        if (DYNAMIC_FETCH && !poolEmpty && __popcll(live) < fetchThreshold) break;
    }
}

template <bool FAST, bool FLAT, int OCT = 8, bool PROLOGUE = false, bool SLICED = false, bool TRIM = false>
__device__ __forceinline__ void traverse_unified(const UnifiedBufs& ub, RayRegs& r, int& node, LaneStack& st,
                                                 int (&spill)[SPILL_DEPTH], bool anyHit, int& hitAddr, float& hitU, float& hitV,
                                                 unsigned int* status, bool poolEmpty, int fetchThreshold, int* slice = nullptr)
{
    if (PROLOGUE && ub.uniformPrologue) uniform_prologue<FAST, OCT, true>(ub, r, node, st, spill, status);
    for (;;) {
        const unsigned long long live = __ballot(node != kSentinel);
        if (live == 0ull) break;
        if (!poolEmpty && __popcll(live) < fetchThreshold) break;
        if (SLICED && --*slice < 0) break;
        float4 a, b, c, d;
        unified_fetch<FLAT, TRIM>(ub, node, live, a, b, c, d);
        if (FLAT && TRIM) { keep_row(a); keep_row(b); keep_row(c); keep_row(d); }
        else if (FLAT) { keep(a); keep(b); keep(c); keep(d); }
        unified_advance<FAST, OCT, LDS_DEPTH, TRIM>(a, b, c, d, r, node, st, spill, anyHit, hitAddr, hitU, hitV, status);
    }
}
__device__ __forceinline__ bool start_ray(const TraceParams& p, int rayIdx, RayRegs& r, int& node, LaneStack& st,
                                          int& hitAddr, float& hitU, float& hitV)
{
    load_ray(p.rays, rayIdx, r);
    hitAddr = -1;
    hitU = hitV = 0.0f;
    stack_reset(st);
    node = (r.tmin < r.tmax) ? 0 : kSentinel;
    return ray_is_nice(r, p.bvhFlags);
}

__device__ __forceinline__ void fresh_prologue(bool fastWave, const UnifiedBufs& ub, const RayRegs& r, int& node, LaneStack& st,
                                               int (&spill)[SPILL_DEPTH], unsigned int* status)
{
    if (fastWave) uniform_prologue<true, 8>(ub, r, node, st, spill, status);
    else uniform_prologue<false, 8>(ub, r, node, st, spill, status);
}

template <bool FLATF>
__device__ __forceinline__ void minipool_body(const TraceParams& p, unsigned int K, lds_int* stackBase);

#define NTR_PERRAY_BOUNDS(W) __launch_bounds__((W) * 64, NTR_TRACE_MIN_WAVES_PER_SIMD)
template <int WAVES, bool STATS, bool UNIFIED = false, bool FLATF = true, bool MINI = false>
__device__ __forceinline__ void perray_body(const TraceParams& p)
{
    __shared__ int s_stack[WAVES][LDS_DEPTH][64];
    if constexpr (MINI) {
        static_assert(WAVES == 1 && UNIFIED && !STATS, "the mini-pool shares the one-wave unified-step launch");
        unsigned int K = (unsigned int)p.poolKConst;
        if (p.poolK) {
            const unsigned int word = *p.poolK;
            if (p.routeSkip == NTR_ROUTE_SKIP_INCOHERENT && NTR_BATCH_WORD_INCOHERENT(word)) return;
            K = NTR_BATCH_WORD_K(word);
        }
        bool pooled = K >= 2u && K <= (unsigned int)NTR_MINIPOOL_MAX_K;
        if (pooled) {
            minipool_body<FLATF>(p, K, (lds_int*)&s_stack[0][0][threadIdx.x]);
            return;
        }
    }
    const int lane = threadIdx.x & 63, wave = threadIdx.x >> 6;
    constexpr int PARTS = 4 / WAVES;
    const unsigned int g = blockIdx.x / PARTS, part = blockIdx.x % PARTS;
    const unsigned int block = p.order ? p.order[g] : g;
    const int rayIdx = block * 256 + part * (WAVES * 64) + threadIdx.x;
    const bool valid = rayIdx < p.numRays;
    const Rsrc nodes = make_rsrc(p.nodes, p.nodesBytes), woop = make_rsrc(p.woop, p.woopBytes);

    unsigned long long tl0 = 0;
    if (p.cost) tl0 = __builtin_amdgcn_s_memrealtime();

    RayRegs r;
    load_ray(p.rays, valid ? rayIdx : 0, r);
    LaneStack st;
    int spill[SPILL_DEPTH];
    st.lds = (lds_int*)&s_stack[wave][0][lane];
    stack_reset(st);

    int hitAddr = -1;
    float hitU = 0.0f, hitV = 0.0f;
    int node = (valid && r.tmin < r.tmax) ? 0 : kSentinel;
    LaneStats ls = {0u, 0u, 0u};

    const bool fastWave = (p.bvhFlags & NTR_BVH_FASTDIV) && __ballot(node != kSentinel && !ray_is_nice(r, p.bvhFlags)) == 0ull;
    int oct = 8;
    if (UNIFIED && fastWave && p.octant && (p.bvhFlags & NTR_BVH_ORDERED)) {
        const unsigned long long liveMask = __ballot(node != kSentinel);
        const unsigned long long sx = __ballot(node != kSentinel && r.dx < 0.0f), sy = __ballot(node != kSentinel && r.dy < 0.0f),
                                 sz = __ballot(node != kSentinel && r.dz < 0.0f);
        if ((sx == 0ull || sx == liveMask) && (sy == 0ull || sy == liveMask) && (sz == 0ull || sz == liveMask))
            oct = (sx ? 1 : 0) | (sy ? 2 : 0) | (sz ? 4 : 0);
    }
    if (UNIFIED) {
        const UnifiedBufs ub = unified_bufs<true>(p);
#define NTR_UNIFIED_OCT(O) traverse_unified<true, FLATF, O, true, false, true>(ub, r, node, st, spill, p.anyHit != 0, hitAddr, hitU, hitV, p.status, true, 0)
        if (oct < 8) {
            switch (oct) {
                case 0: NTR_UNIFIED_OCT(0); break;
                case 1: NTR_UNIFIED_OCT(1); break;
                case 2: NTR_UNIFIED_OCT(2); break;
                case 3: NTR_UNIFIED_OCT(3); break;
                case 4: NTR_UNIFIED_OCT(4); break;
                case 5: NTR_UNIFIED_OCT(5); break;
                case 6: NTR_UNIFIED_OCT(6); break;
                default: NTR_UNIFIED_OCT(7); break;
            }
        }
#undef NTR_UNIFIED_OCT
        else if (fastWave) traverse_unified<true, FLATF, 8, true, false, true>(ub, r, node, st, spill, p.anyHit != 0, hitAddr, hitU, hitV, p.status, true, 0);
        else traverse_unified<false, FLATF, 8, true, false, true>(ub, r, node, st, spill, p.anyHit != 0, hitAddr, hitU, hitV, p.status, true, 0);
    } else if (fastWave) traverse<true, STATS, false>(nodes, woop, r, node, st, spill, p.anyHit != 0, hitAddr, hitU, hitV, ls, p.status, true, 0, p.leafSwitchBelow);
    else traverse<false, STATS, false>(nodes, woop, r, node, st, spill, p.anyHit != 0, hitAddr, hitU, hitV, ls, p.status, true, 0, p.leafSwitchBelow);

    if (p.cost && lane == 0)
        atomicMax(&p.cost[block], (unsigned int)(__builtin_amdgcn_s_memrealtime() - tl0));
    if (!valid) return;
    store_result(p.results, p.triIndex, rayIdx, hitAddr, r.tmax, hitU, hitV);
    if (STATS) {
        atomicAdd(&p.stats[0], (unsigned long long)ls.inner);
        atomicAdd(&p.stats[1], (unsigned long long)ls.tris);
        atomicAdd(&p.stats[2], (unsigned long long)ls.leaves);
        atomicAdd(&p.stats[3], (unsigned long long)(hitAddr >= 0));
    }
}

template <int WAVES, bool STATS, bool UNIFIED = false, bool FLATF = true>
__global__ NTR_PERRAY_BOUNDS(WAVES) void trace_bvh_perray(TraceParams p)
{
    perray_body<WAVES, STATS, UNIFIED, FLATF, false>(p);
}
#define NTR_MINI_BOUNDS __launch_bounds__(64)
__global__ NTR_MINI_BOUNDS void trace_bvh_perray_mini(TraceParams p)
{
    perray_body<1, false, true, true, true>(p);
}
__global__ NTR_MINI_BOUNDS void trace_bvh_perray_mini_desc(TraceParams p)
{
    perray_body<1, false, true, false, true>(p);
}

template <int WAVES, bool UNIFIED = false, bool FLATF = true>
__global__ __launch_bounds__(WAVES * 64, NTR_TRACE_PERSISTENT_MIN_WAVES_PER_SIMD) void trace_bvh_persistent(TraceParams p)
{
    __shared__ int s_stack[WAVES][LDS_DEPTH][64];
    const int lane = threadIdx.x & 63, wave = threadIdx.x >> 6;
    const Rsrc nodes = make_rsrc(p.nodes, p.nodesBytes), woop = make_rsrc(p.woop, p.woopBytes);
    const bool anyHit = p.anyHit != 0;
    const bool bvhFast = (p.bvhFlags & NTR_BVH_FASTDIV) != 0;
    int numBlocksEff = p.numBlocks;
    const unsigned int batchWord = p.poolK ? *p.poolK : 1u;
    const bool incoherentBatch = NTR_BATCH_WORD_INCOHERENT(batchWord);
    if (p.routeSkip == NTR_ROUTE_SKIP_COHERENT && !incoherentBatch) return;
    const int gridIncoherent = NTR_BATCH_WORD_K(batchWord) > 1u ? p.numBlocksIncoherent : p.numBlocksDivergent;
    if (incoherentBatch && gridIncoherent > 0 && gridIncoherent < numBlocksEff) numBlocksEff = gridIncoherent;
    if ((int)blockIdx.x >= numBlocksEff) return;

    LaneStack st;
    int spill[SPILL_DEPTH];
    st.lds = (lds_int*)&s_stack[wave][0][lane];
    stack_reset(st);

    RayRegs r = {0, 0, 0, 0, 0, 0, 0, 0, 0, 0, 0};
    int node = kSentinel, rayIdx = -1, hitAddr = -1;
    float hitU = 0.0f, hitV = 0.0f;
    bool nice = true;
    int chunkNext = 0, chunkEnd = 0;
    bool poolEmpty = false;
    const int numHeads = p.numHeads;
    int shard = (int)(blockIdx.x % (unsigned)numHeads);
    bool firstChunk = true;
    const unsigned int* const order = p.order;
    const int poolEnd = numHeads * p.shardRays;
    auto range_beg = [&](int h) { return h * p.shardRays; };
    int chunkDelta = 0;
    auto chunk_delta = [&](int base, int h) {
        const int off = base - h * p.shardRays;
        if (!order) return ((off / p.chunk) * numHeads + h) * p.chunk - base;
        const int q = (off >> 8) * numHeads + h;
        if (q >= p.orderBlocks) return 0x3FFFFFFF - base;
        return (int)order[q] * 256 + (off & 255) - base;
    };
    auto static_rays = [&](int h) { return ((numBlocksEff - h + numHeads - 1) / numHeads) * WAVES * p.chunk; };
    LaneStats ls = {0u, 0u, 0u};
    SplitState split;
    split_reset(split);
    bool splitOn = false;
    const int splitSlice = UNIFIED ? p.splitSlice : 0;

    const bool dynamicFetch = p.fetchThreshold > 0 && (!UNIFIED || p.wholeWave == 0 || incoherentBatch);
    int prefetched = 0;
    bool havePrefetch = false;
    int prefetchHead = 0;
    int prefetchIn = -1;
    int costBlock = -1;
    unsigned long long costT0 = 0;

    auto grab = [&]() -> bool {
        bool got = false;
        auto take = [&](int base, int h) {
            const int rangeBeg = range_beg(h);
            const int rangeEnd = min(rangeBeg + p.shardRays, poolEnd);
            if (base >= rangeEnd) return false;
            chunkNext = base;
            chunkEnd = min(base + p.chunk, rangeEnd);
            chunkDelta = chunk_delta(base, h);
            return true;
        };
        if (firstChunk) {
            firstChunk = false;
            got = take(range_beg(shard) + ((int)(blockIdx.x / (unsigned)numHeads) * WAVES + __builtin_amdgcn_readfirstlane(wave)) * p.chunk, shard);
        } else if (havePrefetch) {
            havePrefetch = false;
            got = take(__builtin_amdgcn_readfirstlane(prefetched) + static_rays(prefetchHead) + range_beg(prefetchHead), prefetchHead);
        }
        while (!got) {
            int base = 0;
            if (lane == 0) base = atomicAdd(p.counter + shard * 16, p.chunk);
            if (take(__builtin_amdgcn_readfirstlane(base) + static_rays(shard) + range_beg(shard), shard)) { got = true; break; }
            unsigned long long live = 0ull;
            int ofs = 1;
            for (; ofs < numHeads && live == 0ull; ofs += 64) {
                bool has = false;
                if (ofs + lane < numHeads) {
                    const int h = (shard + ofs + lane) % numHeads;
                    const int hb = range_beg(h);
                    const int he = min(hb + p.shardRays, poolEnd);
                    const int taken = __hip_atomic_load(p.counter + h * 16, __ATOMIC_RELAXED, __HIP_MEMORY_SCOPE_AGENT);
                    has = hb + static_rays(h) + taken < he;
                }
                live = __ballot(has);
            }
            if (live == 0ull) break;
            shard = (shard + ofs - 64 + (int)__builtin_ctzll(live)) % numHeads;
        }
        if (got) prefetchIn = p.prefetchAfter;
        return got;
    };
    auto cost_open = [&]() {
        costBlock = (chunkEnd - p.chunk + chunkDelta) >> 8;
        if ((unsigned)costBlock >= (unsigned)((p.numRays + 255) >> 8)) costBlock = -1;
        costT0 = __builtin_amdgcn_s_memrealtime();
    };

    for (;;) {
        unsigned long long empty = __ballot(rayIdx < 0);
        const bool wholeWave = empty == ~0ull;
        const bool refill = !poolEmpty && (wholeWave || (dynamicFetch && 64 - __popcll(empty) < p.fetchThreshold));
        while (refill && empty != 0ull && !poolEmpty) {
            if (chunkNext >= chunkEnd && !grab()) { poolEmpty = true; break; }
            const int prefix = lane_rank(empty);
            const int avail = chunkEnd - chunkNext;
            const int pos = chunkNext + prefix + chunkDelta;
            if (rayIdx < 0 && prefix < avail && pos < p.numRays) {
                rayIdx = pos;
                nice = start_ray(p, rayIdx, r, node, st, hitAddr, hitU, hitV);
            }
            chunkNext += min(__popcll(empty), avail);
            empty = __ballot(rayIdx < 0);
            if (wholeWave && !dynamicFetch) break;
        }
        const bool fresh = refill && wholeWave;
        if (p.cost && refill && wholeWave && !dynamicFetch && !poolEmpty) cost_open();

        if (UNIFIED && poolEmpty && splitSlice > 0) {
            if (!splitOn) { splitOn = true; split_reset(split); }
            split_donate(split, r, node, st, rayIdx, hitAddr, hitU, hitV, nice);
        }
        const bool fastWave = bvhFast && __ballot(node != kSentinel && !nice) == 0ull;
        int slice = 0x7FFFFFFF;
        if (splitOn) slice = splitSlice;
        else if (prefetchIn >= 0 && !poolEmpty) slice = prefetchIn;
        const int fetchBelow = dynamicFetch ? p.fetchThreshold : 0;
        if (UNIFIED) {
            const UnifiedBufs ub = unified_bufs(p);
            if (fresh && p.uniformPrologue) fresh_prologue(fastWave, ub, r, node, st, spill, p.status);
            if (fastWave) traverse_unified<true, FLATF, 8, false, true>(ub, r, node, st, spill, anyHit, hitAddr, hitU, hitV, p.status, poolEmpty, fetchBelow, &slice);
            else traverse_unified<false, FLATF, 8, false, true>(ub, r, node, st, spill, anyHit, hitAddr, hitU, hitV, p.status, poolEmpty, fetchBelow, &slice);
            if (splitOn) split_settle(split, r, node, st, hitAddr, hitU, hitV, anyHit);
        } else {
            if (fresh && p.uniformPrologue) fresh_prologue(fastWave, unified_bufs(p), r, node, st, spill, p.status);
            if (fastWave) traverse<true, false, true, true>(nodes, woop, r, node, st, spill, anyHit, hitAddr, hitU, hitV, ls, p.status, poolEmpty, fetchBelow, p.leafSwitchBelow, &slice);
            else traverse<false, false, true, true>(nodes, woop, r, node, st, spill, anyHit, hitAddr, hitU, hitV, ls, p.status, poolEmpty, fetchBelow, p.leafSwitchBelow, &slice);
        }
        if (!splitOn && prefetchIn >= 0 && !poolEmpty) {
            prefetchIn = -1;
            if (!havePrefetch && __ballot(node != kSentinel) != 0ull) {
                if (lane == 0) prefetched = atomicAdd(p.counter + shard * 16, p.chunk);
                havePrefetch = true;
                prefetchHead = shard;
            }
        }

        if (rayIdx >= 0 && node == kSentinel && (!splitOn || split.base == 0)) {
            store_result(p.results, p.triIndex, rayIdx, hitAddr, r.tmax, hitU, hitV);
            rayIdx = -1;
        }
        if (costBlock >= 0 && __ballot(rayIdx >= 0) == 0ull) {
            if (lane == 0) atomicMax(&p.cost[costBlock], (unsigned int)(__builtin_amdgcn_s_memrealtime() - costT0));
            costBlock = -1;
        }
        if (poolEmpty && __ballot(rayIdx >= 0) == 0ull) break;
    }
}

template <bool FLATF>
__device__ __forceinline__ void minipool_body(const TraceParams& p, unsigned int K, lds_int* stackBase)
{
    const int lane = threadIdx.x;
    const unsigned int numChunks = gridDim.x;
    const unsigned int q = blockIdx.x / K;
    const unsigned int members = min(K, numChunks - q * K);
    if (blockIdx.x - q * K != ((((q * 0x9E3779B1u) >> 16) * members) >> 16)) return;
    unsigned int chunk = q * K;
    const unsigned int chunkEnd = min(chunk + K, numChunks);
    if (chunk >= chunkEnd) return;
    unsigned int block = p.order ? p.order[chunk >> 2] : (chunk >> 2);
    int poolNext = (int)(block * 256u + (chunk & 3u) * 64u);
    int poolEnd = min(poolNext + 64, p.numRays);
    const bool anyHit = p.anyHit != 0;
    const bool bvhFast = (p.bvhFlags & NTR_BVH_FASTDIV) != 0;
    const UnifiedBufs ub = unified_bufs<true>(p);

    unsigned long long tl0 = 0;
    if (p.cost) tl0 = __builtin_amdgcn_s_memrealtime();

    LaneStack st;
    int spill[SPILL_DEPTH];
    st.lds = stackBase;
    stack_reset(st);
    RayRegs r = {0, 0, 0, 0, 0, 0, 0, 0, 0, 0, 0};
    int node = kSentinel, rayIdx = -1, hitAddr = -1;
    float hitU = 0.0f, hitV = 0.0f;
    bool nice = true;

    for (;;) {
        while (poolNext >= poolEnd && chunk + 1u < chunkEnd) {
            chunk++;
            block = p.order ? p.order[chunk >> 2] : (chunk >> 2);
            poolNext = (int)(block * 256u + (chunk & 3u) * 64u);
            poolEnd = min(poolNext + 64, p.numRays);
        }
        const unsigned long long empty = __ballot(rayIdx < 0);
        if (empty != 0ull && poolNext < poolEnd) {
            const int prefix = lane_rank(empty);
            const int avail = poolEnd - poolNext;
            if (rayIdx < 0 && prefix < avail) {
                rayIdx = poolNext + prefix;
                nice = start_ray(p, rayIdx, r, node, st, hitAddr, hitU, hitV);
            }
            poolNext += min(__popcll(empty), avail);
        }
        const bool poolEmpty = poolNext >= poolEnd && chunk + 1u >= chunkEnd;
        const bool fastWave = bvhFast && __ballot(node != kSentinel && !nice) == 0ull;
        if (fastWave) traverse_unified<true, FLATF, 8, false, false, true>(ub, r, node, st, spill, anyHit, hitAddr, hitU, hitV, p.status, poolEmpty, p.fetchThreshold);
        else traverse_unified<false, FLATF, 8, false, false, true>(ub, r, node, st, spill, anyHit, hitAddr, hitU, hitV, p.status, poolEmpty, p.fetchThreshold);
        if (rayIdx >= 0 && node == kSentinel) {
            store_result(p.results, p.triIndex, rayIdx, hitAddr, r.tmax, hitU, hitV);
            rayIdx = -1;
        }
        if (poolEmpty && __ballot(rayIdx >= 0) == 0ull) break;
    }
    if (p.cost && lane == 0) {
        const unsigned int life = (unsigned int)(__builtin_amdgcn_s_memrealtime() - tl0);
        for (unsigned int c = q * K; c < chunkEnd; c += 4u - (c & 3u)) atomicMax(&p.cost[p.order ? p.order[c >> 2] : (c >> 2)], life);
    }
}

}

extern "C" hipError_t ntr_launch_trace(int variant, const ntr::TraceParams* p, int numBlocks, hipStream_t stream)
{
    constexpr int WAVES = NTR_TRACE_WAVES_PER_BLOCK;
    switch (variant) {
    case NTR_VARIANT_PERRAY_UNIFIED_W1:
        if (p->flatFetch) hipLaunchKernelGGL((ntr::trace_bvh_perray<1, false, true, true>), dim3(numBlocks), dim3(64), 0, stream, *p);
        else hipLaunchKernelGGL((ntr::trace_bvh_perray<1, false, true, false>), dim3(numBlocks), dim3(64), 0, stream, *p);
        break;
    case NTR_VARIANT_PERRAY_UNIFIED_MINI:
        if (p->flatFetch) hipLaunchKernelGGL(ntr::trace_bvh_perray_mini, dim3(numBlocks), dim3(64), 0, stream, *p);
        else hipLaunchKernelGGL(ntr::trace_bvh_perray_mini_desc, dim3(numBlocks), dim3(64), 0, stream, *p);
        break;
    case NTR_VARIANT_PERRAY_STATS:
        hipLaunchKernelGGL((ntr::trace_bvh_perray<WAVES, true>), dim3(numBlocks), dim3(WAVES * 64), 0, stream, *p);
        break;
    case NTR_VARIANT_PERSISTENT_UNIFIED:
        if (p->flatFetch) hipLaunchKernelGGL((ntr::trace_bvh_persistent<WAVES, true, true>), dim3(numBlocks), dim3(WAVES * 64), 0, stream, *p);
        else hipLaunchKernelGGL((ntr::trace_bvh_persistent<WAVES, true, false>), dim3(numBlocks), dim3(WAVES * 64), 0, stream, *p);
        break;
    case NTR_VARIANT_PERSISTENT:
        hipLaunchKernelGGL((ntr::trace_bvh_persistent<WAVES, false>), dim3(numBlocks), dim3(WAVES * 64), 0, stream, *p);
        break;
    default:
        return hipErrorInvalidValue;
    }
    return hipGetLastError();
}
```

### ntrace_amd/csrc/trace_lane.h

```cpp
#pragma once
#include <hip/hip_runtime.h>
#include <stdint.h>
#include <float.h>

#include "trace_kernels.h"
#include "trace_arith.h"
#include "trace_fetch.h"

namespace ntr {

static constexpr int LDS_DEPTH = 16;
static constexpr int SPILL_DEPTH = 88;

__device__ __forceinline__ float sel_min(float a, float b) { return (a < b) ? a : b; }
__device__ __forceinline__ float sel_max(float a, float b) { return (a > b) ? a : b; }

struct RayRegs {
    float ox, oy, oz, tmin;
    float dx, dy, dz, tmax;
    float rx, ry, rz;
};

__device__ __forceinline__ bool nice_dir(float v) { const float a = fabsf(v); return a >= 0x1p-40f && a <= 0x1p20f; }
__device__ __forceinline__ bool nice_pos(float v, bool zeroOk)
{
    const float a = fabsf(v);
    return (a >= 0x1p-36f && a < 0x1p55f) || (zeroOk && v == 0.0f);
}
__device__ __forceinline__ bool ray_is_nice(const RayRegs& r, uint32_t bvhFlags)
{
    const bool zeroOk = (bvhFlags & NTR_BVH_NOTINY) != 0;
    return nice_dir(r.dx) && nice_dir(r.dy) && nice_dir(r.dz) && nice_pos(r.ox, zeroOk) && nice_pos(r.oy, zeroOk) &&
           nice_pos(r.oz, zeroOk);
}
template <bool FAST, int OCT = 8>
__device__ __forceinline__ void ray_box2(const RayRegs& r, const float4& n0, const float4& n1, const float4& nz,
                                         float& mn0, float& mx0, float& mn1, float& mx1)
{
    if (FAST) {
        float x[12] = {n0.x - r.ox, n0.y - r.ox, n0.z - r.oy, n0.w - r.oy, nz.x - r.oz, nz.y - r.oz,
                       n1.x - r.ox, n1.y - r.ox, n1.z - r.oy, n1.w - r.oy, nz.z - r.oz, nz.w - r.oz};
        const float d[3] = {r.dx, r.dy, r.dz};
        const float rc[3] = {r.rx, r.ry, r.rz};
        float q[12], e[12];
#pragma unroll
        for (int k = 0; k < 12; k++) q[k] = x[k] * rc[(k % 6) >> 1];
#pragma unroll
        for (int k = 0; k < 12; k++) e[k] = __builtin_fmaf(-d[(k % 6) >> 1], q[k], x[k]);
#pragma unroll
        for (int k = 0; k < 12; k++) q[k] = __builtin_fmaf(e[k], rc[(k % 6) >> 1], q[k]);
        if (OCT < 8) {
            constexpr int sx = OCT & 1, sy = (OCT >> 1) & 1, sz = (OCT >> 2) & 1;
            mn0 = fmaxf(fmaxf(q[0 + sx], q[2 + sy]), q[4 + sz]);
            mx0 = fminf(fminf(q[1 - sx], q[3 - sy]), q[5 - sz]);
            mn1 = fmaxf(fmaxf(q[6 + sx], q[8 + sy]), q[10 + sz]);
            mx1 = fminf(fminf(q[7 - sx], q[9 - sy]), q[11 - sz]);
        } else {
            mn0 = fmaxf(fmaxf(fminf(q[0], q[1]), fminf(q[2], q[3])), fminf(q[4], q[5]));
            mx0 = fminf(fminf(fmaxf(q[0], q[1]), fmaxf(q[2], q[3])), fmaxf(q[4], q[5]));
            mn1 = fmaxf(fmaxf(fminf(q[6], q[7]), fminf(q[8], q[9])), fminf(q[10], q[11]));
            mx1 = fminf(fminf(fmaxf(q[6], q[7]), fmaxf(q[8], q[9])), fmaxf(q[10], q[11]));
        }
    } else {
        float t0x = (n0.x - r.ox) / r.dx, t1x = (n0.y - r.ox) / r.dx;
        float t0y = (n0.z - r.oy) / r.dy, t1y = (n0.w - r.oy) / r.dy;
        float t0z = (nz.x - r.oz) / r.dz, t1z = (nz.y - r.oz) / r.dz;
        mn0 = sel_max(sel_max(sel_min(t0x, t1x), sel_min(t0y, t1y)), sel_min(t0z, t1z));
        mx0 = sel_min(sel_min(sel_max(t0x, t1x), sel_max(t0y, t1y)), sel_max(t0z, t1z));
        t0x = (n1.x - r.ox) / r.dx; t1x = (n1.y - r.ox) / r.dx;
        t0y = (n1.z - r.oy) / r.dy; t1y = (n1.w - r.oy) / r.dy;
        t0z = (nz.z - r.oz) / r.dz; t1z = (nz.w - r.oz) / r.dz;
        mn1 = sel_max(sel_max(sel_min(t0x, t1x), sel_min(t0y, t1y)), sel_min(t0z, t1z));
        mx1 = sel_min(sel_min(sel_max(t0x, t1x), sel_max(t0y, t1y)), sel_max(t0z, t1z));
    }
}

__device__ __forceinline__ float dot4(float4 a, float bx, float by, float bz, float bw)
{
    float r = 0.0f;
    r += a.x * bx;
    r += a.y * by;
    r += a.z * bz;
    r += a.w * bw;
    return r;
}

typedef __attribute__((address_space(3))) int lds_int;

struct LaneStack {
    lds_int* lds;
    int sp;
    int tos;
};

__device__ __forceinline__ void stack_reset(LaneStack& st) { st.sp = 0; st.tos = kSentinel; }

template <int LD = LDS_DEPTH>
__device__ __forceinline__ void stack_push(LaneStack& st, int (&spill)[SPILL_DEPTH], int v, unsigned int* status)
{
    if (__builtin_expect(st.sp < LD, 1)) st.lds[st.sp * 64] = st.tos;
    else if (st.sp < LD + SPILL_DEPTH) spill[st.sp - LD] = st.tos;
    else { atomicOr(status, NTR_STATUS_STACK_OVERFLOW); return; }
    st.sp++;
    st.tos = v;
}
template <int LD = LDS_DEPTH>
__device__ __forceinline__ int stack_pop(LaneStack& st, int (&spill)[SPILL_DEPTH])
{
    const int r = st.tos;
    if (st.sp > 0) {
        st.sp--;
        st.tos = __builtin_expect(st.sp < LD, 1) ? st.lds[st.sp * 64] : spill[st.sp - LD];
    } else {
        st.tos = kSentinel;
    }
    return r;
}

template <int LD = LDS_DEPTH>
__device__ __forceinline__ int stack_pop_flat(LaneStack& st, int (&spill)[SPILL_DEPTH])
{
    const int r = st.tos;
    if (st.sp > 0) {
        st.sp--;
        int v = st.lds[min(st.sp, LD - 1) * 64];
        if (__builtin_expect(st.sp >= LD, 0)) v = spill[st.sp - LD];
        st.tos = v;
    }
    return r;
}

__device__ __forceinline__ void keep(float4& v) { asm volatile("" : "+v"(v.x), "+v"(v.y), "+v"(v.z), "+v"(v.w)); }
__device__ __forceinline__ void keep(unsigned int& v) { asm volatile("" : "+v"(v)); }
__device__ __forceinline__ void keep_row(float4& v) { u32x4 t = as_u4(v); asm volatile("" : "+v"(t)); v = as_f4(t); }

__device__ __forceinline__ int lane_rank(unsigned long long m)
{
    return __builtin_amdgcn_mbcnt_hi((unsigned)(m >> 32), __builtin_amdgcn_mbcnt_lo((unsigned)m, 0));
}

struct LaneStats {
    unsigned int inner, tris, leaves;
};

static constexpr int kNoNode = (int)0xFFFFFF00u;

__device__ __forceinline__ void load_ray(const NtrRay* __restrict__ rays, int rayIdx, RayRegs& r)
{
    const float4 o = reinterpret_cast<const float4*>(rays)[rayIdx * 2 + 0];
    const float4 d = reinterpret_cast<const float4*>(rays)[rayIdx * 2 + 1];
    r.ox = o.x; r.oy = o.y; r.oz = o.z; r.tmin = o.w;
    r.dx = d.x; r.dy = d.y; r.dz = d.z; r.tmax = d.w;
    r.rx = exact_rcp(d.x); r.ry = exact_rcp(d.y); r.rz = exact_rcp(d.z);
}

__device__ __forceinline__ void store_result(NtrRayResult* __restrict__ results, const int* __restrict__ triIndex,
                                             int rayIdx, int hitAddr, float t, float u, float v)
{
    int4 out;
    out.x = (hitAddr < 0) ? -1 : triIndex[hitAddr];
    out.y = __float_as_int(t);
    out.z = (hitAddr < 0) ? 0 : __float_as_int(u);
    out.w = (hitAddr < 0) ? 0 : __float_as_int(v);
    reinterpret_cast<int4*>(results)[rayIdx] = out;
}

template <bool FAST, int OCT, int LD = LDS_DEPTH, bool TRIM = false>
__device__ __forceinline__ void inner_advance(const float4& a, const float4& b, const float4& c, const float4& d, const RayRegs& r, int& node,
                                              LaneStack& st, int (&spill)[SPILL_DEPTH], unsigned int* status)
{
    float mn0, mx0, mn1, mx1;
    ray_box2<FAST, OCT>(r, a, b, c, mn0, mx0, mn1, mx1);
    const bool i0 = (mn0 <= mx0) && (mx0 >= r.tmin) && (mn0 <= r.tmax);
    const bool i1 = (mn1 <= mx1) && (mx1 >= r.tmin) && (mn1 <= r.tmax);
    const int c0 = __float_as_int(d.x), c1 = __float_as_int(d.y);
    const bool swp = i1 && (!i0 || mn0 > mn1);
    const int nearC = swp ? c1 : c0, farC = swp ? c0 : c1;
    if (i0 && i1) stack_push<LD>(st, spill, farC, status);
    node = (i0 || i1) ? nearC : TRIM ? stack_pop_flat<LD>(st, spill) : stack_pop<LD>(st, spill);
}

template <bool FAST>
__device__ __forceinline__ void inner_step(Rsrc nodes, bool inner, const RayRegs& r,
                                           int& node, LaneStack& st, int (&spill)[SPILL_DEPTH], unsigned int* status)
{
    const int ofs = inner ? node : kNoNode;
    const float4 n0 = ld4(nodes, ofs), n1 = ld4(nodes, ofs + kRowBytes), nz = ld4(nodes, ofs + 2 * kRowBytes);
    float4 nc = ld4(nodes, ofs + 3 * kRowBytes);
    keep(nc);
    if (inner) inner_advance<FAST, 8>(n0, n1, nz, nc, r, node, st, spill, status);
}

__device__ __forceinline__ bool triangle_step(const float4& z, const float4& u4, const float4& v4, RayRegs& r, float& hitU, float& hitV)
{
    const float Oz = z.w - r.ox * z.x - r.oy * z.y - r.oz * z.z;
    const float ooDz = 1.0f / dot4(z, r.dx, r.dy, r.dz, 0.0f);
    const float t = Oz * ooDz;
    float tt = FLT_MAX, uu = 0.0f, vv = 0.0f;
    if (t > r.tmin && t < r.tmax) {
        const float u = dot4(u4, r.ox, r.oy, r.oz, 1.0f) + t * dot4(u4, r.dx, r.dy, r.dz, 0.0f);
        if (u >= 0.0f) {
            const float v = dot4(v4, r.ox, r.oy, r.oz, 1.0f) + t * dot4(v4, r.dx, r.dy, r.dz, 0.0f);
            if (v >= 0.0f && (u + v) <= 1.0f) { tt = t; uu = u; vv = v; }
        }
    }
    const bool hit = tt > r.tmin && tt < r.tmax;
    if (hit) { r.tmax = tt; hitU = uu; hitV = vv; }
    return hit;
}

template <bool STATS>
__device__ __forceinline__ bool leaf_step(Rsrc woop, RayRegs& r, int leaf, bool anyHit, int& hitAddr,
                                          float& hitU, float& hitV, LaneStats& ls)
{
    for (int ofs = leaf_row(leaf) * kRowBytes;; ofs += kTriBytes) {
        const float4 z = ld4(woop, ofs);
        float4 u4 = ld4(woop, ofs + kRowBytes);
        float4 v4 = ld4(woop, ofs + 2 * kRowBytes);
        unsigned int nextWord = ld1(woop, ofs + kTriBytes);
        keep(u4); keep(v4); keep(nextWord);
        if (__float_as_uint(z.x) == kLeafTerm) {
            if (STATS) ls.leaves++;
            break;
        }
        if (STATS) ls.tris++;

        const int row = ofs >> kRowShift;
        if (triangle_step(z, u4, v4, r, hitU, hitV)) {
            hitAddr = row;
            if (anyHit) return true;
        }
        if (nextWord == kLeafTerm) {
            if (STATS) ls.leaves++;
            break;
        }
    }
    return false;
}

template <bool FAST, int OCT, int LD = LDS_DEPTH, bool TRIM = false>
__device__ __forceinline__ void unified_advance(const float4& a, const float4& b, const float4& c, const float4& d, RayRegs& r, int& node,
                                                LaneStack& st, int (&spill)[SPILL_DEPTH], bool anyHit, int& hitAddr, float& hitU, float& hitV,
                                                unsigned int* status)
{
    const bool inner = (unsigned)node < (unsigned)kSentinel;
    const bool atTri = node < 0;
    if (inner) {
        inner_advance<FAST, OCT, LD, TRIM>(a, b, c, d, r, node, st, spill, status);
    } else if (atTri) {
        bool leafDone = __float_as_uint(a.x) == kLeafTerm;
        if (!leafDone) {
            bool terminated = false;
            if (triangle_step(a, b, c, r, hitU, hitV)) {
                hitAddr = leaf_row(node);
                terminated = anyHit;
            }
            if (terminated) node = kSentinel;
            else if (__float_as_uint(d.x) == kLeafTerm) leafDone = true;
            else node -= kTriRows;
        }
        if (leafDone) node = TRIM ? stack_pop_flat<LD>(st, spill) : stack_pop<LD>(st, spill);
    }
}

}
```

### ntrace_amd/csrc/trace_prologue.h

```cpp
#pragma once
#include "trace_lane.h"

namespace ntr {

typedef float f32x4 __attribute__((ext_vector_type(4)));
typedef const __attribute__((address_space(4))) f32x4* const_f32x4_ptr;

static constexpr int kCertainGiveUpAfter = 2;

__device__ __forceinline__ float certain_reach(float tmax, float d)
{
    const float p = tmax * fabsf(d);
    return (p >= 0x1p-100f) ? p * 0x1.00001p0f : __builtin_inff();
}
template <int SIGN>
__device__ __forceinline__ float certain_end(float o, float reach)
{
    const float s = SIGN > 0 ? o + reach : o - reach;
    return __builtin_fmaf(fabsf(s), SIGN > 0 ? 0x1p-22f : -0x1p-22f, s);
}

__device__ __forceinline__ int certain_masks(f32x4 A, f32x4 B, f32x4 C, int c0, int c1, const RayRegs& r, float loX, float hiX, float loY, float hiY,
                                             float loZ, float hiZ, unsigned long long live, unsigned long long& in0, unsigned long long& in1,
                                             unsigned long long& reach)
{
    unsigned long long sav;
    int next;
    asm volatile(
        "s_mov_b64 %[sav], exec\n\t"
        "s_mov_b32 %[next], %[none]\n\t"
        "s_and_b64 exec, %[sav], %[live]\n\t"
        "v_cmpx_le_f32 vcc, %[ax], %[ox]\n\t"
        "v_cmpx_ge_f32 vcc, %[ay], %[ox]\n\t"
        "v_cmpx_le_f32 vcc, %[az], %[oy]\n\t"
        "v_cmpx_ge_f32 vcc, %[aw], %[oy]\n\t"
        "v_cmpx_le_f32 vcc, %[cx], %[oz]\n\t"
        "v_cmpx_ge_f32 vcc, %[cy], %[oz]\n\t"
        "s_mov_b64 %[in0], exec\n\t"
        "s_cmp_eq_u64 %[in0], %[live]\n\t"
        "s_cbranch_scc0 .Lcs_g%=\n\t"
        "s_mov_b64 %[in1], 0\n\t"
        "v_cmpx_le_f32 vcc, %[bx], %[hx]\n\t"
        "v_cmpx_ge_f32 vcc, %[by], %[lx]\n\t"
        "v_cmpx_le_f32 vcc, %[bz], %[hy]\n\t"
        "v_cmpx_ge_f32 vcc, %[bw], %[ly]\n\t"
        "v_cmpx_le_f32 vcc, %[cz], %[hz]\n\t"
        "v_cmpx_ge_f32 vcc, %[cw], %[lz]\n\t"
        "s_mov_b64 %[reach], exec\n\t"
        "s_cbranch_execnz .Lcs_e%=\n\t"
        "s_mov_b32 %[next], %[c0]\n\t"
        "s_branch .Lcs_e%=\n"
        ".Lcs_g%=:\n\t"
        "s_and_b64 exec, %[sav], %[live]\n\t"
        "s_andn2_b64 exec, exec, %[in0]\n\t"
        "s_cbranch_execz .Lcs_a%=\n\t"
        "v_cmpx_le_f32 vcc, %[bx], %[ox]\n\t"
        "v_cmpx_ge_f32 vcc, %[by], %[ox]\n\t"
        "v_cmpx_le_f32 vcc, %[bz], %[oy]\n\t"
        "v_cmpx_ge_f32 vcc, %[bw], %[oy]\n\t"
        "v_cmpx_le_f32 vcc, %[cz], %[oz]\n\t"
        "v_cmpx_ge_f32 vcc, %[cw], %[oz]\n\t"
        "s_cbranch_execz .Lcs_a%=\n\t"
        "s_mov_b64 %[in1], exec\n\t"
        "v_cmpx_le_f32 vcc, %[ax], %[hx]\n\t"
        "v_cmpx_ge_f32 vcc, %[ay], %[lx]\n\t"
        "v_cmpx_le_f32 vcc, %[az], %[hy]\n\t"
        "v_cmpx_ge_f32 vcc, %[aw], %[ly]\n\t"
        "v_cmpx_le_f32 vcc, %[cx], %[hz]\n\t"
        "v_cmpx_ge_f32 vcc, %[cy], %[lz]\n\t"
        "s_mov_b64 %[reach], exec\n\t"
        "s_branch .Lcs_b%=\n"
        ".Lcs_a%=:\n\t"
        "s_mov_b64 %[in1], 0\n\t"
        "s_mov_b64 %[reach], 0\n"
        ".Lcs_b%=:\n\t"
        "s_mov_b64 exec, %[in0]\n\t"
        "s_cbranch_execz .Lcs_c%=\n\t"
        "v_cmpx_le_f32 vcc, %[bx], %[hx]\n\t"
        "v_cmpx_ge_f32 vcc, %[by], %[lx]\n\t"
        "v_cmpx_le_f32 vcc, %[bz], %[hy]\n\t"
        "v_cmpx_ge_f32 vcc, %[bw], %[ly]\n\t"
        "v_cmpx_le_f32 vcc, %[cz], %[hz]\n\t"
        "v_cmpx_ge_f32 vcc, %[cw], %[lz]\n\t"
        "s_or_b64 %[reach], %[reach], exec\n"
        ".Lcs_c%=:\n\t"
        "s_cmp_eq_u64 %[in1], %[live]\n\t"
        "s_cbranch_scc0 .Lcs_e%=\n\t"
        "s_cmp_eq_u64 %[reach], 0\n\t"
        "s_cselect_b32 %[next], %[c1], %[next]\n"
        ".Lcs_e%=:\n\t"
        "s_mov_b64 exec, %[sav]"
        : [sav] "=&s"(sav), [in0] "=&s"(in0), [in1] "=&s"(in1), [reach] "=&s"(reach), [next] "=&s"(next)
        : [live] "s"(live), [ax] "s"(A.x), [ay] "s"(A.y), [az] "s"(A.z), [aw] "s"(A.w), [bx] "s"(B.x), [by] "s"(B.y), [bz] "s"(B.z), [bw] "s"(B.w),
          [cx] "s"(C.x), [cy] "s"(C.y), [cz] "s"(C.z), [cw] "s"(C.w), [c0] "s"(c0), [c1] "s"(c1), [none] "i"(kSentinel), [ox] "v"(r.ox), [oy] "v"(r.oy),
          [oz] "v"(r.oz), [lx] "v"(loX), [hx] "v"(hiX), [ly] "v"(loY), [hy] "v"(hiY), [lz] "v"(loZ), [hz] "v"(hiZ)
        : "vcc", "scc");
    return next;
}
__device__ __forceinline__ void take_children(int& node, int c0, int c1, unsigned long long m0, unsigned long long m1)
{
    unsigned long long sav;
    asm volatile(
        "s_mov_b64 %[sav], exec\n\t"
        "s_mov_b64 exec, %[m1]\n\t"
        "v_mov_b32 %[node], %[c1]\n\t"
        "s_mov_b64 exec, %[m0]\n\t"
        "v_mov_b32 %[node], %[c0]\n\t"
        "s_mov_b64 exec, %[sav]"
        : [sav] "=&s"(sav), [node] "+v"(node)
        : [m0] "s"(m0), [m1] "s"(m1), [c0] "s"(c0), [c1] "s"(c1));
}

template <bool FAST, int OCT, bool CERTAIN = false>
__device__ __forceinline__ void uniform_prologue(const UnifiedBufs& ub, const RayRegs& r, int& node, LaneStack& st, int (&spill)[SPILL_DEPTH],
                                                 unsigned int* status)
{
    if ((reinterpret_cast<unsigned long long>(ub.nodes) & (unsigned long long)(kNodeBytes - 1)) != 0ull) return;
    bool tryCertain = false;
    int uncertain = 0;
    float loX = 0.0f, hiX = 0.0f, loY = 0.0f, hiY = 0.0f, loZ = 0.0f, hiZ = 0.0f;
    if (CERTAIN && FAST) {
        tryCertain = ub.certainSteps && __ballot(node != kSentinel && r.tmin != 0.0f) == 0ull;
        if (tryCertain) {
            const float fx = certain_reach(r.tmax, r.dx), fy = certain_reach(r.tmax, r.dy), fz = certain_reach(r.tmax, r.dz);
            loX = r.dx < 0.0f ? certain_end<-1>(r.ox, fx) : r.ox; hiX = r.dx < 0.0f ? r.ox : certain_end<1>(r.ox, fx);
            loY = r.dy < 0.0f ? certain_end<-1>(r.oy, fy) : r.oy; hiY = r.dy < 0.0f ? r.oy : certain_end<1>(r.oy, fy);
            loZ = r.dz < 0.0f ? certain_end<-1>(r.oz, fz) : r.oz; hiZ = r.dz < 0.0f ? r.oz : certain_end<1>(r.oz, fz);
        }
    }
    unsigned int descentLim = !ub.certainDescent ? 0u : ub.nodesBytes - (unsigned)kNodeBytes < (unsigned)kSentinel ? ub.nodesBytes - (unsigned)kNodeBytes : (unsigned)kSentinel - 1u;
    asm volatile("" : "+s"(descentLim));
    for (;;) {
        const bool live = node != kSentinel;
        const unsigned long long liveMask = __ballot(live);
        if (liveMask == 0ull) return;
        const int unode = __builtin_amdgcn_readlane(node, (int)__builtin_ctzll(liveMask));
        if (__ballot(live && node != unode) != 0ull) return;
        if ((unsigned)unode >= (unsigned)kSentinel || (unsigned)unode > ub.nodesBytes - (unsigned)kNodeBytes) return;
        unsigned int snode = (unsigned)unode;
        f32x4 A, B, C, D;
        if (CERTAIN && FAST && tryCertain) {
            unsigned long long in0, in1, reach;
            for (;;) {
                const const_f32x4_ptr q = (const_f32x4_ptr)(ub.nodes + snode);
                A = q[0]; B = q[1]; C = q[2]; D = q[3];
                const int next = certain_masks(A, B, C, __float_as_int(D.x), __float_as_int(D.y), r, loX, hiX, loY, hiY, loZ, hiZ, liveMask, in0, in1, reach);
                if ((unsigned)next - 1u >= descentLim) break;
                snode = (unsigned)next;
            }
            if (snode != (unsigned)unode) {
                if (live) node = (int)snode;
                uncertain = 0;
            }
            if ((in0 | in1) == liveMask && reach == 0ull) {
                take_children(node, __float_as_int(D.x), __float_as_int(D.y), in0, in1);
                uncertain = 0;
                continue;
            }
            if (++uncertain >= kCertainGiveUpAfter) tryCertain = false;
        } else {
            const const_f32x4_ptr q = (const_f32x4_ptr)(ub.nodes + snode);
            A = q[0]; B = q[1]; C = q[2]; D = q[3];
        }
        if (live)
            inner_advance<FAST, OCT>(make_float4(A.x, A.y, A.z, A.w), make_float4(B.x, B.y, B.z, B.w), make_float4(C.x, C.y, C.z, C.w),
                                     make_float4(D.x, D.y, D.z, D.w), r, node, st, spill, status);
    }
}

}
```

Before: 17240.

## Precompute trace constants on host and add quirk-free triangle fast path

Adds a TraceConsts block, filled on the host, that carries buffer resource words, limits, descent bound and feature switches, so the unified kernel setup reads them instead of deriving them per wave. Replaces the per-lane nice-ray predicate with a branchless integer ray_class test and reuses one live-mask ballot. Adds a QUIRK=false triangle test that skips the FLT_MAX temporary path when no lane in the wave has a non-finite tmax. Also adds a selftest kernel that checks the new classifier against the old rule. The cost is more template instantiations and larger code, plus the risk that the new classifier disagrees with the old one on edge cases.

```diff
diff --git a/include/ntrace_amd.h b/include/ntrace_amd.h
--- a/include/ntrace_amd.h
+++ b/include/ntrace_amd.h
@@ -181,6 +181,7 @@
 NTR_API int ntr_selftest_division(const float* d_x, int32_t nx, const float* d_d, int32_t nd,
                                   uint32_t* mismatches, void* stream);
 NTR_API int ntr_selftest_division_hard(int32_t xExp, int32_t dExp, uint64_t* pairs, uint64_t* mismatches, void* stream);
+NTR_API int ntr_selftest_ray_class(const NtrRay* d_rays, int32_t numRays, uint32_t bvhFlags, uint32_t* mismatches, void* stream);
 
 
 NTR_API int ntr_pixel_table(int32_t w, int32_t h, int32_t* d_indexToPixel, int32_t* d_pixelToIndex, void* stream);
diff --git a/ntrace_amd/__init__.py b/ntrace_amd/__init__.py
--- a/ntrace_amd/__init__.py
+++ b/ntrace_amd/__init__.py
@@ -1,6 +1,6 @@
 from ._capi import (BvhView, RAY_DTYPE, RESULT_DTYPE, HostBvh, KernelConfig, NtrError, TraceStats, bvh_validate, lib,
                     lib_path, query_config, sah_build, trace_bvh, trace_bvh_stats, pixel_table,
-                    raygen_primary, raygen_ao, raygen_shadow, count_hits, selftest_division, selftest_division_hard, bvh_leaf_depths, secondary_block_costs, lbvh_capacity,
+                    raygen_primary, raygen_ao, raygen_shadow, count_hits, selftest_division, selftest_division_hard, selftest_ray_class, bvh_leaf_depths, secondary_block_costs, lbvh_capacity,
                     lbvh_build, LbvhResult, hlbvh_build, HlbvhResult, reconstruct, ray_morton_sort, camera_decode, camera_reencode,
                     camera_nscreen_to_world, obj_load, SchedHint, trace_status, trace_plan, trace_plan_hint_step, trace_plan_certain, TracePlan, set_tunables, host_bvh_wrap, use_library, trace_graph_reserve, trace_graph_release_all, stream_release, selftest_auto_hint_table, selftest_gather_rate, frame_shard, frame_ao_batches, DistGroup,
                     lbvh_release_workspace, predict_block_costs, predict_batch_coherence, predict_dispatch_order, SchedHintState,
@@ -26,7 +26,7 @@
            "tesla_persistent_speculative_while_while", "kepler_dynamic_fetch")
 
 __all__ = ["BvhView", "RAY_DTYPE", "RESULT_DTYPE", "HostBvh", "KernelConfig", "NtrError", "bvh_validate", "lib",
-           "lib_path", "query_config", "sah_build", "trace_bvh", "trace_bvh_stats", "TraceStats", "pixel_table", "raygen_primary", "raygen_ao", "count_hits", "selftest_division", "selftest_division_hard", "bvh_leaf_depths", "secondary_block_costs", "lbvh_capacity", "lbvh_build", "LbvhResult", "hlbvh_build", "HlbvhResult", "reconstruct", "ray_morton_sort", "camera_decode", "camera_reencode", "camera_nscreen_to_world", "obj_load", "SchedHint", "trace_status", "set_tunables", "host_bvh_wrap", "BVHLayout_Compact", "KERNELS",
+           "lib_path", "query_config", "sah_build", "trace_bvh", "trace_bvh_stats", "TraceStats", "pixel_table", "raygen_primary", "raygen_ao", "count_hits", "selftest_division", "selftest_division_hard", "selftest_ray_class", "bvh_leaf_depths", "secondary_block_costs", "lbvh_capacity", "lbvh_build", "LbvhResult", "hlbvh_build", "HlbvhResult", "reconstruct", "ray_morton_sort", "camera_decode", "camera_reencode", "camera_nscreen_to_world", "obj_load", "SchedHint", "trace_status", "set_tunables", "host_bvh_wrap", "BVHLayout_Compact", "KERNELS",
            "HostKdtree", "kdtree_build", "host_kdtree_wrap", "trace_kdtree", "KDTREE_SPATIAL_MEDIAN", "KDTREE_SAH",
            "DeviceKdtree", "KdtreeDeviceParams", "kdtree_device_build", "kdtree_device_params", "KDTREE_DEVICE_DEFAULTS",
            "kdtree_device_scratch_bytes", "PersistentBvhParams", "PersistentBvhResult", "persistent_bvh_params",
diff --git a/ntrace_amd/_capi.py b/ntrace_amd/_capi.py
--- a/ntrace_amd/_capi.py
+++ b/ntrace_amd/_capi.py
@@ -330,6 +330,7 @@
     ("ntr_bvh_leaf_depths", C.c_int, [_vp, _i64, _vp, _i64, _vp, _i32, _vp, C.POINTER(_i32), _vp]),
     ("ntr_selftest_division", C.c_int, [_vp, _i32, _vp, _i32, C.POINTER(_u32), _vp]),
     ("ntr_selftest_division_hard", C.c_int, [_i32, _i32, C.POINTER(C.c_uint64), C.POINTER(C.c_uint64), _vp]),
+    ("ntr_selftest_ray_class", C.c_int, [_vp, _i32, _u32, C.POINTER(_u32), _vp]),
     ("ntr_trace_bvh_stats", C.c_int, [C.c_char_p, _i32, _i32, _vp, _vp, _vp, _i64, _vp, _i64, _vp, _i32, _u32, _vp,
                                       C.POINTER(TraceStats)]),
     ("ntr_bvh_validate", C.c_int, [_vp, _i64, C.POINTER(_u32), _vp]),
@@ -682,6 +683,12 @@
     return int(n.value), int(m.value)
 
 
+def selftest_ray_class(d_rays, num_rays, bvh_flags, stream=0):
+    m = _u32(0)
+    _check(lib().ntr_selftest_ray_class(_vp(d_rays), int(num_rays), int(bvh_flags), C.byref(m), _vp(stream)))
+    return int(m.value)
+
+
 def trace_bvh_stats(kernel, num_rays, any_hit, d_rays, d_results, d_nodes, nodes_bytes, d_woop, woop_bytes,
                     d_tri_index, layout=4, bvh_flags=0, stream=0):
     st = TraceStats()
diff --git a/ntrace_amd/csrc/ntr_api.cpp b/ntrace_amd/csrc/ntr_api.cpp
--- a/ntrace_amd/csrc/ntr_api.cpp
+++ b/ntrace_amd/csrc/ntr_api.cpp
@@ -94,6 +94,24 @@
     TopTable* predTable = nullptr;
     PredictScratch* predScratch = nullptr;
 };
+
+static void trace_fill_consts(TraceParams& p)
+{
+    TraceConsts& k = p.k;
+    const unsigned long long an = (unsigned long long)p.nodes, aw = (unsigned long long)p.woop, lo = an < aw ? an : aw;
+    k.base = (const char*)lo;
+    k.dN = (uint32_t)(an - lo); k.dW = (uint32_t)(aw - lo);
+    k.limNode = p.nodesBytes - (uint32_t)kNodeBytes;
+    k.limTri = leaf_link((int)((p.woopBytes - (uint32_t)kNodeBytes) >> kRowShift));
+    k.oddBase = k.limNode + 1u; k.oddSpan = (uint32_t)k.limTri - k.oddBase;
+    k.rNodes[0] = (uint32_t)an; k.rNodes[1] = (uint32_t)(an >> 32) & 0xFFFFu; k.rNodes[2] = p.nodesBytes; k.rNodes[3] = 0x00020000u;
+    k.rWoop[0] = (uint32_t)aw; k.rWoop[1] = (uint32_t)(aw >> 32) & 0xFFFFu; k.rWoop[2] = p.woopBytes; k.rWoop[3] = 0x00020000u;
+    k.descentLim = !p.certainDescent ? 0u : k.limNode < (uint32_t)kSentinel ? k.limNode : (uint32_t)kSentinel - 1u;
+    const bool ordered = (p.bvhFlags & NTR_BVH_ORDERED) != 0;
+    k.switches = ((p.bvhFlags & NTR_BVH_FASTDIV) ? NTR_K_FAST : 0u) | ((p.bvhFlags & NTR_BVH_NOTINY) ? NTR_K_ZERO_ORIGIN : 0u) |
+                 ((p.octant && ordered) ? NTR_K_OCTANT : 0u) | ((p.certainSteps && ordered) ? NTR_K_CERTAIN : 0u) |
+                 ((p.uniformPrologue && (an & (unsigned long long)(kNodeBytes - 1)) == 0ull) ? NTR_K_PROLOGUE : 0u);
+}
 
 static int bind_trace(DeviceState* ds, const Tunables& tun, const TracePlan& pl, bool capturing, int64_t nodesBytes, hipStream_t s,
                       NtrSchedHint* hint, TraceLaunch* L)
@@ -166,6 +184,8 @@
         p.routeSkip = NTR_ROUTE_SKIP_INCOHERENT;
         if (variant == NTR_VARIANT_PERSISTENT) { p.fetchThreshold = pl.perrayFetchThreshold; p.poolKConst = 1; }
     }
+    trace_fill_consts(p);
+    trace_fill_consts(pp);
     return NTR_OK;
 }
 
@@ -648,6 +668,23 @@
     return NTR_OK;
 }
 
+int ntr_selftest_ray_class(const NtrRay* d_rays, int32_t numRays, uint32_t bvhFlags, uint32_t* mismatches, void* stream)
+{
+    if (!mismatches || !d_rays || numRays <= 0) return set_error(NTR_ERR_INVALID, "ntr_selftest_ray_class: bad argument");
+    hipStream_t s = (hipStream_t)stream;
+    unsigned int* d_m = nullptr;
+    NTR_HIP(hipMalloc((void**)&d_m, sizeof(unsigned int)));
+    hipError_t e = hipMemsetAsync(d_m, 0, sizeof(unsigned int), s);
+    if (e == hipSuccess) e = ntr_launch_selftest_ray_class(d_rays, numRays, bvhFlags, d_m, s);
+    unsigned int m = 0;
+    if (e == hipSuccess) e = hipMemcpyAsync(&m, d_m, sizeof(m), hipMemcpyDeviceToHost, s);
+    if (e == hipSuccess) e = hipStreamSynchronize(s);
+    (void)hipFree(d_m);
+    if (e != hipSuccess) return hip_fail(e, "ntr_selftest_ray_class");
+    *mismatches = m;
+    return NTR_OK;
+}
+
 int ntr_selftest_division_hard(int32_t xExp, int32_t dExp, uint64_t* pairs, uint64_t* mismatches, void* stream)
 {
     if (!pairs || !mismatches || xExp < -84 || xExp > 51 || dExp < -40 || dExp > 16)
diff --git a/ntrace_amd/csrc/selftest_kernels.hip b/ntrace_amd/csrc/selftest_kernels.hip
--- a/ntrace_amd/csrc/selftest_kernels.hip
+++ b/ntrace_amd/csrc/selftest_kernels.hip
@@ -3,6 +3,7 @@
 
 #include "trace_kernels.h"
 #include "trace_arith.h"
+#include "trace_lane.h"
 
 namespace ntr {
 
@@ -63,6 +64,24 @@
     if (bad) atomicAdd(&counts[1], bad);
 }
 
+__global__ __launch_bounds__(256) void selftest_ray_class_kernel(const NtrRay* __restrict__ rays, int numRays, uint32_t bvhFlags,
+                                                                 unsigned int* __restrict__ mismatches)
+{
+    const int i = blockIdx.x * blockDim.x + threadIdx.x;
+    if (i >= numRays) return;
+    const float4 o = reinterpret_cast<const float4*>(rays)[i * 2 + 0], d = reinterpret_cast<const float4*>(rays)[i * 2 + 1];
+    RayRegs r = {o.x, o.y, o.z, o.w, d.x, d.y, d.z, d.w, 0.0f, 0.0f, 0.0f};
+    const bool rule = ray_is_nice(r, bvhFlags);
+    const bool fast = ray_class(r, nice_zero_word(bvhFlags)) <= kNiceMax;
+    if (rule != fast) atomicAdd(mismatches, 1u);
+}
+
+}
+
+extern "C" hipError_t ntr_launch_selftest_ray_class(const NtrRay* d_rays, int numRays, uint32_t bvhFlags, unsigned int* d_mismatches, hipStream_t stream)
+{
+    hipLaunchKernelGGL(ntr::selftest_ray_class_kernel, dim3((numRays + 255) / 256), dim3(256), 0, stream, d_rays, numRays, bvhFlags, d_mismatches);
+    return hipGetLastError();
 }
 
 extern "C" hipError_t ntr_launch_selftest_division(const float* d_x, const float* d_d, int nx, int nd,
diff --git a/ntrace_amd/csrc/trace_fetch.h b/ntrace_amd/csrc/trace_fetch.h
--- a/ntrace_amd/csrc/trace_fetch.h
+++ b/ntrace_amd/csrc/trace_fetch.h
@@ -88,6 +88,7 @@
     unsigned int limNode;
     int limTri;
     unsigned int oddBase, oddSpan;
+    unsigned int descentLim;
 };
 template <bool TRIM = false>
 __device__ __forceinline__ UnifiedBufs unified_bufs(const TraceParams& p)
@@ -95,6 +96,16 @@
     UnifiedBufs u;
     u.nodes = (const char*)p.nodes; u.woop = (const char*)p.woop;
     u.nodesBytes = p.nodesBytes; u.woopBytes = p.woopBytes;
+    if (TRIM) {
+        const TraceConsts& k = p.k;
+        u.rNodes = u32x4{k.rNodes[0], k.rNodes[1], k.rNodes[2], k.rNodes[3]}; u.rWoop = u32x4{k.rWoop[0], k.rWoop[1], k.rWoop[2], k.rWoop[3]};
+        u.uniformPrologue = (k.switches & NTR_K_PROLOGUE) != 0u;
+        u.certainSteps = (k.switches & NTR_K_CERTAIN) != 0u;
+        u.certainDescent = k.descentLim != 0u;
+        u.base = k.base; u.dN = k.dN; u.dW = k.dW; u.limNode = k.limNode; u.limTri = k.limTri;
+        u.oddBase = k.oddBase; u.oddSpan = k.oddSpan; u.descentLim = k.descentLim;
+        return u;
+    }
     u.rNodes = rsrc_words(p.nodes, p.nodesBytes); u.rWoop = rsrc_words(p.woop, p.woopBytes);
     u.uniformPrologue = p.uniformPrologue != 0;
     u.certainSteps = p.certainSteps != 0 && (p.bvhFlags & NTR_BVH_ORDERED) != 0;
diff --git a/ntrace_amd/csrc/trace_kernels.h b/ntrace_amd/csrc/trace_kernels.h
--- a/ntrace_amd/csrc/trace_kernels.h
+++ b/ntrace_amd/csrc/trace_kernels.h
@@ -31,6 +31,22 @@
 
 
 namespace ntr {
+
+#define NTR_K_FAST 1u
+#define NTR_K_ZERO_ORIGIN 2u
+#define NTR_K_OCTANT 4u
+#define NTR_K_CERTAIN 8u
+#define NTR_K_PROLOGUE 16u
+struct TraceConsts {
+    const char* base;
+    uint32_t dN, dW;
+    uint32_t limNode;
+    int32_t limTri;
+    uint32_t oddBase, oddSpan;
+    uint32_t rNodes[4], rWoop[4];
+    uint32_t descentLim;
+    uint32_t switches;
+};
 
 struct TraceParams {
     int32_t numRays;
@@ -68,6 +84,7 @@
     const unsigned int* poolK;
     int32_t poolKConst;
     int32_t routeSkip;
+    TraceConsts k;
 };
 
 }
@@ -98,3 +115,4 @@
 extern "C" hipError_t ntr_launch_selftest_division(const float* d_x, const float* d_d, int nx, int nd,
                                                    unsigned int* d_mismatches, hipStream_t stream);
 extern "C" hipError_t ntr_launch_selftest_division_hard(int xe0, int de0, unsigned long long* d_counts, hipStream_t stream);
+extern "C" hipError_t ntr_launch_selftest_ray_class(const NtrRay* d_rays, int numRays, uint32_t bvhFlags, unsigned int* d_mismatches, hipStream_t stream);
diff --git a/ntrace_amd/csrc/trace_kernels.hip b/ntrace_amd/csrc/trace_kernels.hip
--- a/ntrace_amd/csrc/trace_kernels.hip
+++ b/ntrace_amd/csrc/trace_kernels.hip
@@ -36,12 +36,12 @@
     }
 }
 
-template <bool FAST, bool FLAT, int OCT = 8, bool PROLOGUE = false, bool SLICED = false, bool TRIM = false>
+template <bool FAST, bool FLAT, int OCT = 8, bool PROLOGUE = false, bool SLICED = false, bool TRIM = false, bool QUIRK = true>
 __device__ __forceinline__ void traverse_unified(const UnifiedBufs& ub, RayRegs& r, int& node, LaneStack& st,
                                                  int (&spill)[SPILL_DEPTH], bool anyHit, int& hitAddr, float& hitU, float& hitV,
                                                  unsigned int* status, bool poolEmpty, int fetchThreshold, int* slice = nullptr)
 {
-    if (PROLOGUE && ub.uniformPrologue) uniform_prologue<FAST, OCT, true>(ub, r, node, st, spill, status);
+    if (PROLOGUE && ub.uniformPrologue) uniform_prologue<FAST, OCT, true, TRIM>(ub, r, node, st, spill, status);
     for (;;) {
         const unsigned long long live = __ballot(node != kSentinel);
         if (live == 0ull) break;
@@ -51,7 +51,7 @@
         unified_fetch<FLAT, TRIM>(ub, node, live, a, b, c, d);
         if (FLAT && TRIM) { keep_row(a); keep_row(b); keep_row(c); keep_row(d); }
         else if (FLAT) { keep(a); keep(b); keep(c); keep(d); }
-        unified_advance<FAST, OCT, LDS_DEPTH, TRIM>(a, b, c, d, r, node, st, spill, anyHit, hitAddr, hitU, hitV, status);
+        unified_advance<FAST, OCT, LDS_DEPTH, TRIM, QUIRK>(a, b, c, d, r, node, st, spill, anyHit, hitAddr, hitU, hitV, status);
     }
 }
 __device__ __forceinline__ bool start_ray(const TraceParams& p, int rayIdx, RayRegs& r, int& node, LaneStack& st,
@@ -101,34 +101,38 @@
     const int rayIdx = block * 256 + part * (WAVES * 64) + threadIdx.x;
     const bool valid = rayIdx < p.numRays;
     const Rsrc nodes = make_rsrc(p.nodes, p.nodesBytes), woop = make_rsrc(p.woop, p.woopBytes);
+    UnifiedBufs ub;
+    if (UNIFIED) ub = unified_bufs<true>(p);
 
     unsigned long long tl0 = 0;
     if (p.cost) tl0 = __builtin_amdgcn_s_memrealtime();
 
-    RayRegs r;
-    load_ray(p.rays, valid ? rayIdx : 0, r);
     LaneStack st;
     int spill[SPILL_DEPTH];
     st.lds = (lds_int*)&s_stack[wave][0][lane];
     stack_reset(st);
+    RayRegs r;
+    load_ray(p.rays, valid ? rayIdx : 0, r);
 
     int hitAddr = -1;
     float hitU = 0.0f, hitV = 0.0f;
-    int node = (valid && r.tmin < r.tmax) ? 0 : kSentinel;
+    const bool live = valid && r.tmin < r.tmax;
+    int node = live ? 0 : kSentinel;
     LaneStats ls = {0u, 0u, 0u};
-
-    const bool fastWave = (p.bvhFlags & NTR_BVH_FASTDIV) && __ballot(node != kSentinel && !ray_is_nice(r, p.bvhFlags)) == 0ull;
-    int oct = 8;
-    if (UNIFIED && fastWave && p.octant && (p.bvhFlags & NTR_BVH_ORDERED)) {
-        const unsigned long long liveMask = __ballot(node != kSentinel);
-        const unsigned long long sx = __ballot(node != kSentinel && r.dx < 0.0f), sy = __ballot(node != kSentinel && r.dy < 0.0f),
-                                 sz = __ballot(node != kSentinel && r.dz < 0.0f);
+    const unsigned long long liveMask = __builtin_amdgcn_ballot_w64(live);
+
+    const bool fastAllowed = (p.k.switches & NTR_K_FAST) != 0u, octantAllowed = (p.k.switches & NTR_K_OCTANT) != 0u;
+    const unsigned int zeroWord = (p.k.switches & NTR_K_ZERO_ORIGIN) ? kPosZero : (kPosZero | 1u);
+    const bool fastWave = fastAllowed && (liveMask & __builtin_amdgcn_ballot_w64(ray_class(r, zeroWord) > kNiceMax)) == 0ull;
+    int oct = wave_may_quirk(r) ? 9 : 8;
+    if (UNIFIED && fastWave && __builtin_expect(oct == 8, 1) && octantAllowed) {
+        const unsigned long long sx = liveMask & __builtin_amdgcn_ballot_w64(r.dx < 0.0f), sy = liveMask & __builtin_amdgcn_ballot_w64(r.dy < 0.0f),
+                                 sz = liveMask & __builtin_amdgcn_ballot_w64(r.dz < 0.0f);
         if ((sx == 0ull || sx == liveMask) && (sy == 0ull || sy == liveMask) && (sz == 0ull || sz == liveMask))
             oct = (sx ? 1 : 0) | (sy ? 2 : 0) | (sz ? 4 : 0);
     }
     if (UNIFIED) {
-        const UnifiedBufs ub = unified_bufs<true>(p);
-#define NTR_UNIFIED_OCT(O) traverse_unified<true, FLATF, O, true, false, true>(ub, r, node, st, spill, p.anyHit != 0, hitAddr, hitU, hitV, p.status, true, 0)
+#define NTR_UNIFIED_OCT(O) traverse_unified<true, FLATF, O, true, false, true, false>(ub, r, node, st, spill, p.anyHit != 0, hitAddr, hitU, hitV, p.status, true, 0)
         if (oct < 8) {
             switch (oct) {
                 case 0: NTR_UNIFIED_OCT(0); break;
@@ -142,6 +146,7 @@
             }
         }
 #undef NTR_UNIFIED_OCT
+        else if (__builtin_expect(fastWave && oct == 8, 1)) traverse_unified<true, FLATF, 8, true, false, true, false>(ub, r, node, st, spill, p.anyHit != 0, hitAddr, hitU, hitV, p.status, true, 0);
         else if (fastWave) traverse_unified<true, FLATF, 8, true, false, true>(ub, r, node, st, spill, p.anyHit != 0, hitAddr, hitU, hitV, p.status, true, 0);
         else traverse_unified<false, FLATF, 8, true, false, true>(ub, r, node, st, spill, p.anyHit != 0, hitAddr, hitU, hitV, p.status, true, 0);
     } else if (fastWave) traverse<true, STATS, false>(nodes, woop, r, node, st, spill, p.anyHit != 0, hitAddr, hitU, hitV, ls, p.status, true, 0, p.leafSwitchBelow);
@@ -387,7 +392,8 @@
         }
         const bool poolEmpty = poolNext >= poolEnd && chunk + 1u >= chunkEnd;
         const bool fastWave = bvhFast && __ballot(node != kSentinel && !nice) == 0ull;
-        if (fastWave) traverse_unified<true, FLATF, 8, false, false, true>(ub, r, node, st, spill, anyHit, hitAddr, hitU, hitV, p.status, poolEmpty, p.fetchThreshold);
+        if (fastWave && !wave_may_quirk(r)) traverse_unified<true, FLATF, 8, false, false, true, false>(ub, r, node, st, spill, anyHit, hitAddr, hitU, hitV, p.status, poolEmpty, p.fetchThreshold);
+        else if (fastWave) traverse_unified<true, FLATF, 8, false, false, true>(ub, r, node, st, spill, anyHit, hitAddr, hitU, hitV, p.status, poolEmpty, p.fetchThreshold);
         else traverse_unified<false, FLATF, 8, false, false, true>(ub, r, node, st, spill, anyHit, hitAddr, hitU, hitV, p.status, poolEmpty, p.fetchThreshold);
         if (rayIdx >= 0 && node == kSentinel) {
             store_result(p.results, p.triIndex, rayIdx, hitAddr, r.tmax, hitU, hitV);
diff --git a/ntrace_amd/csrc/trace_lane.h b/ntrace_amd/csrc/trace_lane.h
--- a/ntrace_amd/csrc/trace_lane.h
+++ b/ntrace_amd/csrc/trace_lane.h
@@ -32,6 +32,17 @@
     const bool zeroOk = (bvhFlags & NTR_BVH_NOTINY) != 0;
     return nice_dir(r.dx) && nice_dir(r.dy) && nice_dir(r.dz) && nice_pos(r.ox, zeroOk) && nice_pos(r.oy, zeroOk) &&
            nice_pos(r.oz, zeroOk);
+}
+static constexpr unsigned int kDirLo2 = 0x57000000u, kDirSpan2 = 0x3C000000u, kPosLo2 = 0x5B000000u, kNiceMax = 0x5AFFFFFEu;
+static constexpr unsigned int kDirPad = kNiceMax - kDirSpan2, kPosZero = 0u - kPosLo2;
+__device__ __forceinline__ unsigned int nice_zero_word(uint32_t bvhFlags) { return (bvhFlags & NTR_BVH_NOTINY) ? kPosZero : (kPosZero | 1u); }
+__device__ __forceinline__ unsigned int ray_class(const RayRegs& r, unsigned int zeroWord)
+{
+    const unsigned int dx = (__float_as_uint(r.dx) << 1) - kDirLo2, dy = (__float_as_uint(r.dy) << 1) - kDirLo2, dz = (__float_as_uint(r.dz) << 1) - kDirLo2;
+    unsigned int px = (__float_as_uint(r.ox) << 1) - kPosLo2, py = (__float_as_uint(r.oy) << 1) - kPosLo2, pz = (__float_as_uint(r.oz) << 1) - kPosLo2;
+    px = px == zeroWord ? 0u : px; py = py == zeroWord ? 0u : py; pz = pz == zeroWord ? 0u : pz;
+    const unsigned int d = max(max(dx, dy), dz), p = max(max(px, py), pz);
+    return max(p, __builtin_elementwise_add_sat(d, kDirPad));
 }
 template <bool FAST, int OCT = 8>
 __device__ __forceinline__ void ray_box2(const RayRegs& r, const float4& n0, const float4& n1, const float4& nz,
@@ -191,11 +202,23 @@
     if (inner) inner_advance<FAST, 8>(n0, n1, nz, nc, r, node, st, spill, status);
 }
 
+template <bool QUIRK = true>
 __device__ __forceinline__ bool triangle_step(const float4& z, const float4& u4, const float4& v4, RayRegs& r, float& hitU, float& hitV)
 {
     const float Oz = z.w - r.ox * z.x - r.oy * z.y - r.oz * z.z;
     const float ooDz = 1.0f / dot4(z, r.dx, r.dy, r.dz, 0.0f);
     const float t = Oz * ooDz;
+    if (!QUIRK) {
+        bool hit = false;
+        if (t > r.tmin && t < r.tmax) {
+            const float u = dot4(u4, r.ox, r.oy, r.oz, 1.0f) + t * dot4(u4, r.dx, r.dy, r.dz, 0.0f);
+            if (u >= 0.0f) {
+                const float v = dot4(v4, r.ox, r.oy, r.oz, 1.0f) + t * dot4(v4, r.dx, r.dy, r.dz, 0.0f);
+                if (v >= 0.0f && (u + v) <= 1.0f) { r.tmax = t; hitU = u; hitV = v; hit = true; }
+            }
+        }
+        return hit;
+    }
     float tt = FLT_MAX, uu = 0.0f, vv = 0.0f;
     if (t > r.tmin && t < r.tmax) {
         const float u = dot4(u4, r.ox, r.oy, r.oz, 1.0f) + t * dot4(u4, r.dx, r.dy, r.dz, 0.0f);
@@ -208,6 +231,7 @@
     if (hit) { r.tmax = tt; hitU = uu; hitV = vv; }
     return hit;
 }
+__device__ __forceinline__ bool wave_may_quirk(const RayRegs& r) { return __builtin_amdgcn_ballot_w64(!(r.tmax <= FLT_MAX)) != 0ull; }
 
 template <bool STATS>
 __device__ __forceinline__ bool leaf_step(Rsrc woop, RayRegs& r, int leaf, bool anyHit, int& hitAddr,
@@ -238,7 +262,7 @@
     return false;
 }
 
-template <bool FAST, int OCT, int LD = LDS_DEPTH, bool TRIM = false>
+template <bool FAST, int OCT, int LD = LDS_DEPTH, bool TRIM = false, bool QUIRK = true>
 __device__ __forceinline__ void unified_advance(const float4& a, const float4& b, const float4& c, const float4& d, RayRegs& r, int& node,
                                                 LaneStack& st, int (&spill)[SPILL_DEPTH], bool anyHit, int& hitAddr, float& hitU, float& hitV,
                                                 unsigned int* status)
@@ -251,7 +275,7 @@
         bool leafDone = __float_as_uint(a.x) == kLeafTerm;
         if (!leafDone) {
             bool terminated = false;
-            if (triangle_step(a, b, c, r, hitU, hitV)) {
+            if (triangle_step<QUIRK>(a, b, c, r, hitU, hitV)) {
                 hitAddr = leaf_row(node);
                 terminated = anyHit;
             }
diff --git a/ntrace_amd/csrc/trace_prologue.h b/ntrace_amd/csrc/trace_prologue.h
--- a/ntrace_amd/csrc/trace_prologue.h
+++ b/ntrace_amd/csrc/trace_prologue.h
@@ -111,11 +111,11 @@
         : [m0] "s"(m0), [m1] "s"(m1), [c0] "s"(c0), [c1] "s"(c1));
 }
 
-template <bool FAST, int OCT, bool CERTAIN = false>
+template <bool FAST, int OCT, bool CERTAIN = false, bool HOSTK = false>
 __device__ __forceinline__ void uniform_prologue(const UnifiedBufs& ub, const RayRegs& r, int& node, LaneStack& st, int (&spill)[SPILL_DEPTH],
                                                  unsigned int* status)
 {
-    if ((reinterpret_cast<unsigned long long>(ub.nodes) & (unsigned long long)(kNodeBytes - 1)) != 0ull) return;
+    if (!HOSTK && (reinterpret_cast<unsigned long long>(ub.nodes) & (unsigned long long)(kNodeBytes - 1)) != 0ull) return;
     bool tryCertain = false;
     int uncertain = 0;
     float loX = 0.0f, hiX = 0.0f, loY = 0.0f, hiY = 0.0f, loZ = 0.0f, hiZ = 0.0f;
@@ -128,15 +128,15 @@
             loZ = r.dz < 0.0f ? certain_end<-1>(r.oz, fz) : r.oz; hiZ = r.dz < 0.0f ? r.oz : certain_end<1>(r.oz, fz);
         }
     }
-    unsigned int descentLim = !ub.certainDescent ? 0u : ub.nodesBytes - (unsigned)kNodeBytes < (unsigned)kSentinel ? ub.nodesBytes - (unsigned)kNodeBytes : (unsigned)kSentinel - 1u;
-    asm volatile("" : "+s"(descentLim));
+    unsigned int descentLim = HOSTK ? ub.descentLim : !ub.certainDescent ? 0u : ub.nodesBytes - (unsigned)kNodeBytes < (unsigned)kSentinel ? ub.nodesBytes - (unsigned)kNodeBytes : (unsigned)kSentinel - 1u;
+    if (!HOSTK) asm volatile("" : "+s"(descentLim));
     for (;;) {
         const bool live = node != kSentinel;
         const unsigned long long liveMask = __ballot(live);
         if (liveMask == 0ull) return;
         const int unode = __builtin_amdgcn_readlane(node, (int)__builtin_ctzll(liveMask));
         if (__ballot(live && node != unode) != 0ull) return;
-        if ((unsigned)unode >= (unsigned)kSentinel || (unsigned)unode > ub.nodesBytes - (unsigned)kNodeBytes) return;
+        if ((unsigned)unode >= (unsigned)kSentinel || (unsigned)unode > (HOSTK ? ub.limNode : ub.nodesBytes - (unsigned)kNodeBytes)) return;
         unsigned int snode = (unsigned)unode;
         f32x4 A, B, C, D;
         if (CERTAIN && FAST && tryCertain) {
```

Result: faster. 17530 (median of 6 runs) (+1.7%).
